# daysun/grid_ndt

Measured on NVIDIA B200. Metric: ndt_map_build_points_per_sec, higher is better.
Workload: dtype f64

## Files before the change

grid_ndt_b200/_lib.py:

```python
import ctypes as C
import os
import subprocess
import sys

from ._abi import Counts, NdtParams, Params, PointCloud2, Registration, XchgInfo, XchgView

HERE = os.path.dirname(os.path.abspath(__file__))
REPO = os.path.dirname(HERE)
LIB_PATH = os.environ.get("GNDT_LIB") or os.path.join(HERE, "libgndt.so")
SOURCES = [os.path.join(HERE, "csrc", f) for f in (
    "gndt_api.cu", "gndt_device.cuh", "gndt_sort.cuh", "gndt_reduce.cuh", "gndt_label.cuh", "gndt_update.cuh",
    "gndt_exchange.cuh", "gndt_graph.cuh", "gndt_scan.cuh", "gndt_ndt.cuh")]
HEADER = os.path.join(REPO, "include", "gndt.h")
LOOKUP_HEADER = os.path.join(REPO, "include", "gndt_lookup.h")

NVCC_FLAGS = ["-O3", "-std=c++17", "-gencode", "arch=compute_100a,code=sm_100a", "-lineinfo",
              "-Xcompiler", "-fPIC", "-shared"]


def build_library(force=False, verbose=False):
    deps = SOURCES + [HEADER, LOOKUP_HEADER]
    if not force and os.path.exists(LIB_PATH) and all(
            os.path.getmtime(LIB_PATH) >= os.path.getmtime(d) for d in deps if os.path.exists(d)):
        return LIB_PATH
    nvcc = os.environ.get("NVCC", "nvcc")
    cmd = [nvcc] + NVCC_FLAGS + ["-o", LIB_PATH, SOURCES[0], "-I" + os.path.join(REPO, "include")]
    if verbose:
        print(" ".join(cmd), file=sys.stderr)
    subprocess.check_call(cmd)
    return LIB_PATH


class GndtError(RuntimeError):
    def __init__(self, status, msg):
        super().__init__(f"gndt status {status}: {msg}")
        self.status = status


_lib = None

_vp, _sz, _i = C.c_void_p, C.c_size_t, C.c_int
SYMBOLS = {
    "gndt_version": (C.c_char_p, []),
    "gndt_last_error": (C.c_char_p, [_vp]),
    "gndt_default_params": (None, [C.POINTER(Params)]),
    "gndt_create": (_i, [C.POINTER(Params), _i, C.POINTER(_vp)]),
    "gndt_destroy": (_i, [_vp]),
    "gndt_set_params": (_i, [_vp, C.POINTER(Params)]),
    "gndt_build": (_i, [_vp, _vp, _sz, _sz, _i, _vp]),
    "gndt_build_msg": (_i, [_vp, C.POINTER(PointCloud2), _vp]),
    "gndt_update": (_i, [_vp, _vp, _sz, _sz, _i, _vp]),
    "gndt_remove": (_i, [_vp, _vp, _sz, _sz, _i, _vp]),
    "gndt_changed_columns": (_i, [_vp, _vp, _sz, _i, C.POINTER(_sz)]),
    "gndt_counts": (_i, [_vp, C.POINTER(Counts)]),
    "gndt_copy_voxels": (_i, [_vp, _vp, _sz, _i, C.POINTER(_sz)]),
    "gndt_copy_slopes": (_i, [_vp, _vp, _sz, _i, C.POINTER(_sz)]),
    "gndt_copy_columns": (_i, [_vp, _vp, _sz, _i, C.POINTER(_sz)]),
    "gndt_device_voxels": (_i, [_vp, C.POINTER(_vp), C.POINTER(_sz)]),
    "gndt_halo_pack": (_i, [_vp, _vp, _vp, _sz, _vp]),
    "gndt_halo_edges": (_i, [_vp, _vp, _vp, _vp]),
    "gndt_apply_strip_offsets": (_i, [_vp, _vp, C.POINTER(C.c_uint64), C.POINTER(C.c_uint32), C.POINTER(C.c_uint32), _i, _vp]),
    "gndt_device_count_ptr": (_i, [_vp, C.POINTER(_vp)]),
    "gndt_device_table_ptr": (_i, [_vp, C.POINTER(_vp), C.POINTER(_sz)]),
    "gndt_build_edges": (_i, [_vp, _vp, _sz, _vp, _sz, _vp]),
    "gndt_copy_edges": (_i, [_vp, _vp, _sz, _vp, _sz, _i, C.POINTER(_sz), C.POINTER(_sz)]),
    "gndt_xchg_create": (_i, [_vp, _i, _i, _sz, _sz, _i, C.POINTER(XchgInfo)]),
    "gndt_xchg_connect": (_i, [_vp, C.POINTER(XchgInfo), _i]),
    "gndt_xchg_run": (_i, [_vp, _vp]),
    "gndt_xchg_stage": (_i, [_vp, _vp]),
    "gndt_xchg_counts_ready": (_i, [_vp]),
    "gndt_xchg_send": (_i, [_vp, _vp]),
    "gndt_xchg_view_get": (_i, [_vp, C.POINTER(XchgView)]),
    "gndt_multi_create": (_i, [C.POINTER(Params), C.POINTER(C.c_int), _i, _sz, _sz, _i, C.POINTER(_vp)]),
    "gndt_multi_destroy": (_i, [_vp]),
    "gndt_multi_build": (_i, [_vp, _vp, _sz, _sz, _i]),
    "gndt_multi_update": (_i, [_vp, _vp, _sz, _sz, _i]),
    "gndt_multi_view": (_i, [_vp, _i, C.POINTER(XchgView)]),
    "gndt_multi_cuts": (_i, [_vp, C.POINTER(C.c_int32), _i]),
    "gndt_multi_handle": (_vp, [_vp, _i]),
    "gndt_multi_last_error": (C.c_char_p, [_vp]),
    "gndt_plan_tiles": (_i, [_vp, _vp, _sz, _sz, _i, _i, C.POINTER(C.c_int32), _vp]),
    "gndt_set_stage_timing": (_i, [_vp, _i]),
    "gndt_stage_ms": (_i, [_vp, C.POINTER(C.c_float)]),
    "gndt_launch_count": (_i, [_vp, C.POINTER(C.c_uint64)]),
    "gndt_fast_div_status": (_i, [_vp, C.POINTER(C.c_int), C.POINTER(C.c_uint64)]),
    "gndt_trans_morton_xyz": (_i, [C.POINTER(C.c_float), C.c_float, C.c_float, C.POINTER(C.c_float),
                                   C.POINTER(C.c_int32), C.POINTER(C.c_int32), C.POINTER(C.c_int32)]),
    "gndt_count_morton": (C.c_uint32, [C.c_uint32, C.c_uint32]),
    "gndt_morton_to_xy": (None, [C.c_uint32, C.POINTER(C.c_uint32), C.POINTER(C.c_uint32)]),
    "gndt_morton_string": (_i, [C.c_int32, C.c_int32, C.c_char_p]),
    "gndt_cell_center": (_i, [C.POINTER(C.c_float), C.c_float, C.c_float, C.c_int32, C.c_int32, C.c_int32,
                              C.POINTER(C.c_float)]),
    "gndt_origin": (_i, [_vp, C.POINTER(C.c_float)]),
    "gndt_default_ndt_params": (None, [C.POINTER(NdtParams)]),
    "gndt_register": (_i, [_vp, _vp, _sz, _sz, _i, C.POINTER(C.c_double), C.POINTER(NdtParams), C.POINTER(Registration), _vp]),
    "gndt_key_layout": (_i, [_vp, C.POINTER(C.c_int)]),
    "gndt_find_column": (C.c_int64, [_vp, _sz, C.c_int32, C.c_int32]),
    "gndt_find_slope": (C.c_int64, [_vp, _sz, _vp, C.c_int32, C.c_int32, C.c_int32]),
    "gndt_neighbor_column": (C.c_int64, [_vp, _sz, C.c_int32, C.c_int32, _i]),
}


def lib():
    global _lib
    if _lib is None:
        if not os.path.exists(LIB_PATH):
            raise GndtError(-2, f"{LIB_PATH} is not built (run __graft_entry__.build()); there is no CPU fallback")
        L = C.CDLL(LIB_PATH)
        for name, (res, args) in SYMBOLS.items():
            fn = getattr(L, name)
            fn.restype, fn.argtypes = res, args
        _lib = L
    return _lib
```

grid_ndt_b200/csrc/gndt_api.cu:

```cuda
#include <algorithm>
#include <cmath>
#include <cstdio>
#include <cstdlib>
#include <cstring>
#include <string>
#include <thread>
#include <vector>

#include "gndt_device.cuh"
#include "gndt_lookup.h"
#include "gndt_label.cuh"
#include "gndt_reduce.cuh"
#include "gndt_sort.cuh"
#include "gndt_update.cuh"
#include "gndt_exchange.cuh"
#include "gndt_graph.cuh"
#include "gndt_ndt.cuh"
#include <unistd.h>

using namespace gndt;

namespace {

thread_local std::string g_create_error;

struct Buffer {
  void *p = nullptr;
  size_t bytes = 0;
};

enum EvId { EV_H2D0, EV_START, EV_KEY, EV_SORT, EV_REDUCE, EV_LABEL, EV_EDGES, EV_COUNT };

struct DivCheck {
  float len = -1.f;
  float rinv = 0.f;
  int ok = 0;
};

struct SmallWords {
  Totals tot;
  u32 n_new;
  struct {
    int have[2];
    u32 done_counter;
  } x;
};
static_assert(sizeof(Totals) == 32 && sizeof(SmallWords) == 48, "SmallWords layout");

}

struct gndt_handle {
  int device = 0;
  gndt_params params;
  std::string err;
  Buffer in_stage, buf_a, buf_b, zero;
  Buffer mom, mom_alt, table, slopes, columns, vfirst, slope_col;
  void *ring = nullptr;
  cudaEvent_t ring_ev[4] = {};
  bool ring_used[4] = {};
  Buffer msg_points;
  Buffer mom_scan, upd_work;
  int pending_fuse = 0;
  size_t pending_points = 0;
  Ctl saved_ctl;
  gndt_params res_params;
  const u32 *changed_dev = nullptr, *changed_count_dev = nullptr;
  size_t n_changed = 0;
  bool n_changed_valid = false;
  Buffer small;
  size_t cap_points = 0, cap_voxels = 0;
  Ctl *ctl = nullptr;
  u32 *hist = nullptr;
  u32 *zhist = nullptr;
  u32 *row_start = nullptr, *row_end = nullptr;
  u32 *lb[2] = {nullptr, nullptr};
  u64 *glb[2] = {nullptr, nullptr};
  Buffer lookback;
  u64 *tile_state = nullptr;
  GroupState *tile_groups = nullptr;
  TileCarry *carry = nullptr;
  u64 *blk_state = nullptr;
  GroupState *blk_groups = nullptr;
  size_t zero_bytes_used = 0;
  size_t sort_tiles = 0, sort_groups = 0, red_tiles = 0, label_blocks = 0;
  Buffer f_zero;
  Buffer g_work, g_off, g_tgt;
  size_t g_slopes = 0, g_targets = 0;
  bool g_valid = false;
  Buffer ndt_vox, ndt_pts, ndt_part;
  double *ndt_host = nullptr;
  bool ndt_ready = false;
  Buffer xbuf;
  XLayout xl = {};
  XPeers xp = {};
  void *x_opened[kMaxRanks] = {};
  int x_what = 0;
  cudaStream_t x_stream = nullptr;
  cudaEvent_t x_ev[2] = {};
  cudaStream_t x_copy[2] = {};
  cudaEvent_t x_ev_counts = nullptr, x_ev_copy = nullptr;
  u32 *x_counts_host = nullptr;
  bool x_staged = false;
  u32 x_epoch = 0;
  bool x_created = false, x_connected = false;
  bool built = false;
  bool counts_valid = false;
  Ctl host_ctl;
  Totals host_tot, saved_tot;
  cudaStream_t last_stream = nullptr;
  cudaEvent_t ev[EV_COUNT] = {};
  bool timed_h2d = false;
  bool stage_timing = false;
  bool stages_valid = false;
  uint64_t launches = 0;
  uint64_t total_points = 0;
  int sm_count = 148;
  int sort_ctas_per_sm[2] = {1, 1};
  DivCheck div[2];
  uint64_t divcheck_values = 0;
};

namespace {

#define GNDT_CUDA(h, call)                                                                   \
  do {                                                                                       \
    cudaError_t e_ = (call);                                                                 \
    if (e_ != cudaSuccess) {                                                                 \
      (h)->err = std::string(#call) + ": " + cudaGetErrorString(e_);                         \
      return GNDT_ERR_CUDA;                                                                  \
    }                                                                                        \
  } while (0)

int ensure(gndt_handle *h, Buffer &b, size_t bytes) {
  if (b.bytes >= bytes) return GNDT_OK;
  if (b.p) GNDT_CUDA(h, cudaFree(b.p));
  b.p = nullptr;
  b.bytes = 0;
  GNDT_CUDA(h, cudaMalloc(&b.p, bytes));
  b.bytes = bytes;
  return GNDT_OK;
}

int ensure_keep(gndt_handle *h, Buffer &b, size_t bytes, size_t keep, cudaStream_t st) {
  if (b.bytes >= bytes) return GNDT_OK;
  void *np = nullptr;
  GNDT_CUDA(h, cudaMalloc(&np, bytes));
  if (b.p && keep) GNDT_CUDA(h, cudaMemcpyAsync(np, b.p, keep, cudaMemcpyDeviceToDevice, st));
  if (b.p) { GNDT_CUDA(h, cudaStreamSynchronize(st)); GNDT_CUDA(h, cudaFree(b.p)); }
  b.p = np;
  b.bytes = bytes;
  return GNDT_OK;
}

size_t align_up(size_t v, size_t a) { return (v + a - 1) / a * a; }

struct Layout {
  size_t bytes = 0;
  size_t take(size_t n) { const size_t o = bytes; bytes = align_up(bytes + n, 256); return o; }
};
template <typename T> T *at(const Buffer &b, size_t off) { return reinterpret_cast<T *>(static_cast<char *>(b.p) + off); }

struct ScanScratch {
  size_t ctl, state, groups;
  ScanScratch(Layout &L, size_t n) {
    const LookbackScratch s = lookback_scratch((n + kScanTile - 1) / kScanTile);
    ctl = L.take(sizeof(ScanCtl));
    state = L.take(s.words * sizeof(u64));
    groups = L.take(s.groups * sizeof(GroupState));
  }
};

template <typename... KArgs, typename... Args>
void launch(gndt_handle *h, bool pdl, void (*kernel)(KArgs...), dim3 grid, dim3 block, size_t smem, cudaStream_t st,
            Args &&...args) {
  cudaLaunchConfig_t cfg = {};
  cfg.gridDim = grid; cfg.blockDim = block; cfg.dynamicSmemBytes = smem; cfg.stream = st;
  cudaLaunchAttribute attr[1];
  attr[0].id = cudaLaunchAttributeProgrammaticStreamSerialization;
  attr[0].val.programmaticStreamSerializationAllowed = 1;
  cfg.attrs = attr;
  cfg.numAttrs = pdl ? 1 : 0;
  cudaLaunchKernelEx(&cfg, kernel, static_cast<KArgs>(args)...);
  h->launches += 1;
}

struct KeepLaunchCount {
  gndt_handle *h;
  uint64_t n;
  explicit KeepLaunchCount(gndt_handle *h_) : h(h_), n(h_->launches) {}
  ~KeepLaunchCount() { h->launches = n; }
};

int upload(gndt_handle *h, Buffer &stage, const void *xyz, size_t bytes, int mem, cudaStream_t st, cudaEvent_t h2d0,
           const float **d_in) {
  *d_in = static_cast<const float *>(xyz);
  if (mem != GNDT_MEM_HOST) return GNDT_OK;
  const int rc = ensure(h, stage, bytes);
  if (rc != GNDT_OK) return rc;
  if (h2d0) GNDT_CUDA(h, cudaEventRecord(h2d0, st));
  GNDT_CUDA(h, cudaMemcpyAsync(stage.p, xyz, bytes, cudaMemcpyHostToDevice, st));
  *d_in = static_cast<const float *>(stage.p);
  return GNDT_OK;
}

float max_abs_offset(float len) {
  auto ok = [len](uint32_t b) {
    float a;
    memcpy(&a, &b, 4);
    volatile float q = a / len;
    return std::ceil((float)q) <= (float)GNDT_MAX_INDEX;
  };
  uint32_t lo = 0, hi = 0x7f7fffffu;
  if (ok(hi)) lo = hi;
  while (lo + 1 < hi) {
    const uint32_t mid = lo + (hi - lo) / 2;
    if (ok(mid)) lo = mid; else hi = mid;
  }
  float a;
  memcpy(&a, &lo, 4);
  return a;
}

DevParams to_dev(const gndt_params &p, size_t cap_voxels) {
  DevParams d;
  d.max_abs[0] = max_abs_offset(p.grid_len);
  d.max_abs[1] = max_abs_offset(p.z_len);
  d.idx_offset = 0;
  d.fast_div = 0;
  d.rinv[0] = d.rinv[1] = 0.f;
  d.grid_len = p.grid_len; d.z_len = p.z_len; d.slope_interval = p.slope_interval;
  d.demand = p.demand; d.min_points = p.min_points;
  d.rough_max = p.rough_max; d.angle_max_deg = p.angle_max_deg; d.reach_height = p.reach_height;
  d.origin_first = p.origin_is_first_point;
  d.origin[0] = p.origin[0]; d.origin[1] = p.origin[1]; d.origin[2] = p.origin[2];
  d.normalize_cov = p.normalize_cov;
  d.tile_lo = p.tile_lo; d.tile_hi = p.tile_hi;
  d.max_voxels = (u32)cap_voxels;
  return d;
}

__global__ void divcheck_kernel(float len, u32 lo_bits, u32 hi_bits, float *rinv_out, unsigned long long *mismatches) {
  const float r = refined_rcp(len);
  if (blockIdx.x == 0 && threadIdx.x == 0) *rinv_out = r;
  unsigned long long bad = 0;
  for (u64 b = (u64)lo_bits + (u64)blockIdx.x * blockDim.x + threadIdx.x; b <= hi_bits; b += (u64)gridDim.x * blockDim.x) {
    const float a = __uint_as_float((u32)b);
    const float exact = ceilf(__fdiv_rn(a, len));
    const float fast = hoisted_div_ceil(a, len, r);
    if (!(exact == fast)) bad++;
  }
  if (bad) atomicAdd(mismatches, bad);
}

int verify_fast_div(gndt_handle *h, float len, DivCheck &out) {
  if (out.len == len) return GNDT_OK;
  out.len = len;
  out.ok = 0;
  out.rinv = 0.f;
  const char *force = getenv("GNDT_EXACT_DIV");
  if (force && force[0] == '1') return GNDT_OK;
  void *scratch = nullptr;
  GNDT_CUDA(h, cudaMalloc(&scratch, 64));
  GNDT_CUDA(h, cudaMemset(scratch, 0, 64));
  uint32_t lo, hi;
  const float top = 2.f * max_abs_offset(len);
  memcpy(&lo, &len, 4);
  memcpy(&hi, &top, 4);
  KeepLaunchCount keep(h);
  launch(h, false, divcheck_kernel, h->sm_count * 8, 256, 0, nullptr, len, lo, hi, (float *)scratch,
         (unsigned long long *)((char *)scratch + 8));
  unsigned long long host[2] = {0, 0};
  cudaError_t e = cudaGetLastError();
  if (e == cudaSuccess) e = cudaMemcpy(host, scratch, 16, cudaMemcpyDeviceToHost);
  cudaFree(scratch);
  if (e != cudaSuccess) { h->err = std::string("divcheck: ") + cudaGetErrorString(e); return GNDT_ERR_CUDA; }
  memcpy(&out.rinv, &host[0], 4);
  out.ok = (host[1] == 0) ? 1 : 0;
  h->divcheck_values += (uint64_t)hi - lo + 1;
  return GNDT_OK;
}

DevParams make_dev(gndt_handle *h, const gndt_params &p, size_t cap_voxels) {
  DevParams d = to_dev(p, cap_voxels);
  d.fast_div = (h->div[0].ok && h->div[1].ok && h->div[0].len == p.grid_len && h->div[1].len == p.z_len) ? 1 : 0;
  d.rinv[0] = h->div[0].rinv;
  d.rinv[1] = h->div[1].rinv;
  return d;
}

int validate_params(const gndt_params *p) {
  if (!p) return GNDT_ERR_INVALID_ARG;
  if (!(p->grid_len > 0.f) || !(p->z_len > 0.f) || !std::isfinite(p->grid_len) || !std::isfinite(p->z_len))
    return GNDT_ERR_INVALID_ARG;
  if (p->demand != GNDT_DEMAND_SLOPE && p->demand != GNDT_DEMAND_TRUE) return GNDT_ERR_INVALID_ARG;
  if (p->min_points < 1) return GNDT_ERR_INVALID_ARG;
  return GNDT_OK;
}

int reserve(gndt_handle *h, size_t n, size_t cap_vox, size_t keep_mom, cudaStream_t st) {
  int rc;
  if ((rc = ensure(h, h->buf_a, n * sizeof(float4))) != GNDT_OK) return rc;
  if ((rc = ensure(h, h->buf_b, n * sizeof(float4))) != GNDT_OK) return rc;
  if ((rc = ensure_keep(h, h->mom, cap_vox * sizeof(VoxMoments), keep_mom, st)) != GNDT_OK) return rc;
  if ((rc = ensure(h, h->table, cap_vox * sizeof(gndt_voxel))) != GNDT_OK) return rc;
  if ((rc = ensure(h, h->slopes, cap_vox * sizeof(gndt_slope))) != GNDT_OK) return rc;
  if ((rc = ensure(h, h->columns, cap_vox * sizeof(gndt_column))) != GNDT_OK) return rc;
  if ((rc = ensure(h, h->vfirst, cap_vox * sizeof(u32))) != GNDT_OK) return rc;
  if ((rc = ensure(h, h->slope_col, cap_vox * sizeof(u32))) != GNDT_OK) return rc;
  if ((rc = ensure(h, h->small, sizeof(SmallWords))) != GNDT_OK) return rc;
  h->cap_points = n;
  h->cap_voxels = cap_vox;
  h->sort_tiles = (n + kSortTile - 1) / kSortTile;
  h->sort_groups = (h->sort_tiles + kSortGroup - 1) / kSortGroup;
  h->red_tiles = (n + kRedTile - 1) / kRedTile;
  h->label_blocks = (cap_vox + kLabelThreads - 1) / kLabelThreads;
  const LookbackScratch red = lookback_scratch(h->red_tiles), fin = lookback_scratch(h->label_blocks);
  Layout Z;
  const size_t o_ctl = Z.take(sizeof(Ctl));
  const size_t o_hist = Z.take((size_t)kMaxPasses * kMaxBins * sizeof(u32));
  const size_t o_zh = Z.take(kZHistBins * sizeof(u32));
  const size_t o_rs = Z.take(65536 * sizeof(u32));
  const size_t o_re = Z.take(65536 * sizeof(u32));
  const size_t o_ts = Z.take(red.words * sizeof(u64));
  const size_t o_tg = Z.take(red.groups * sizeof(GroupState));
  const size_t o_ca = Z.take(h->red_tiles * sizeof(TileCarry));
  const size_t o_bs = Z.take(fin.words * sizeof(u64));
  const size_t o_bg = Z.take(fin.groups * sizeof(GroupState));
  if ((rc = ensure(h, h->zero, Z.bytes)) != GNDT_OK) return rc;
  h->ctl = at<Ctl>(h->zero, o_ctl);
  h->hist = at<u32>(h->zero, o_hist);
  h->zhist = at<u32>(h->zero, o_zh);
  h->row_start = at<u32>(h->zero, o_rs);
  h->row_end = at<u32>(h->zero, o_re);
  h->tile_state = at<u64>(h->zero, o_ts);
  h->tile_groups = at<GroupState>(h->zero, o_tg);
  h->carry = at<TileCarry>(h->zero, o_ca);
  h->blk_state = at<u64>(h->zero, o_bs);
  h->blk_groups = at<GroupState>(h->zero, o_bg);
  h->zero_bytes_used = Z.bytes;
  Layout B;
  const size_t lb_bytes = h->sort_tiles * kMaxBins * sizeof(u32) + 256, glb_bytes = h->sort_groups * kMaxBins * sizeof(u64) + 256;
  const size_t o_lb[2] = {B.take(lb_bytes), B.take(lb_bytes)}, o_glb[2] = {B.take(glb_bytes), B.take(glb_bytes)};
  if ((rc = ensure(h, h->lookback, B.bytes)) != GNDT_OK) return rc;
  for (int k = 0; k < 2; ++k) {
    h->lb[k] = at<u32>(h->lookback, o_lb[k]);
    h->glb[k] = at<u64>(h->lookback, o_glb[k]);
  }
  return GNDT_OK;
}

int grid_for(const gndt_handle *h, size_t work_items, int per_block, int max_waves) {
  size_t blocks = (work_items + per_block - 1) / per_block;
  size_t cap = (size_t)h->sm_count * max_waves;
  if (blocks > cap) blocks = cap;
  if (blocks < 1) blocks = 1;
  return (int)blocks;
}

int sync_counts(gndt_handle *h) {
  if (!h->built) { h->err = "no map has been built on this handle"; return GNDT_ERR_STATE; }
  if (h->counts_valid) return GNDT_OK;
  GNDT_CUDA(h, cudaMemcpyAsync(&h->host_ctl, h->ctl, sizeof(Ctl), cudaMemcpyDeviceToHost, h->last_stream));
  GNDT_CUDA(h, cudaMemcpyAsync(&h->host_tot, h->small.p, sizeof(Totals), cudaMemcpyDeviceToHost, h->last_stream));
  GNDT_CUDA(h, cudaStreamSynchronize(h->last_stream));
  if (h->pending_fuse) {
    const int sign = h->pending_fuse;
    h->pending_fuse = 0;
    if (h->host_ctl.err) {
      const u32 e = h->host_ctl.err;
      h->host_ctl = h->saved_ctl;
      h->host_tot = h->saved_tot;
      GNDT_CUDA(h, cudaMemcpyAsync(h->ctl, &h->saved_ctl, sizeof(Ctl), cudaMemcpyHostToDevice, h->last_stream));
      GNDT_CUDA(h, cudaMemcpyAsync(h->small.p, &h->saved_tot, sizeof(Totals), cudaMemcpyHostToDevice, h->last_stream));
      GNDT_CUDA(h, cudaStreamSynchronize(h->last_stream));
      h->counts_valid = true;
      if (e & kErrWatchdog) { h->err = "device watchdog tripped (look-back / TMA wait never resolved)"; return GNDT_ERR_INTERNAL; }
      if (e & kErrUnmatched) { h->err = "gndt_remove: the scan holds points that were never fused into the map; map unchanged"; return GNDT_ERR_STATE; }
      h->err = "voxel table capacity (max_voxels) exceeded; map unchanged";
      return GNDT_ERR_CAPACITY;
    }
    std::swap(h->mom, h->mom_alt);
    if (sign > 0) h->total_points += h->pending_points;
    else h->total_points -= h->pending_points;
    u32 nc = 0;
    GNDT_CUDA(h, cudaMemcpy(&nc, h->changed_count_dev, 4, cudaMemcpyDeviceToHost));
    h->n_changed = nc;
    h->n_changed_valid = true;
  }
  if (h->host_ctl.err & kErrWatchdog) { h->err = "device watchdog tripped (look-back / TMA wait never resolved)"; return GNDT_ERR_INTERNAL; }
  if (h->host_ctl.err & kErrCapacity) { h->err = "voxel table capacity (max_voxels) exceeded"; return GNDT_ERR_CAPACITY; }
  h->counts_valid = true;
  return GNDT_OK;
}

int front_end(gndt_handle *h, cudaStream_t st, const float *d_in, size_t n, size_t stride_f, size_t start,
              const DevParams &dp, VoxMoments *out) {
  GNDT_CUDA(h, cudaMemsetAsync(h->zero.p, 0, h->zero_bytes_used, st));
  const size_t tiles = (n + kSortTile - 1) / kSortTile, groups = (tiles + kSortGroup - 1) / kSortGroup;
  auto *bounds = dp.fast_div ? bounds_kernel<true> : bounds_kernel<false>;
  launch(h, true, bounds, grid_for(h, n, 256 * 4, 8), 256, 0, st, h->ctl, h->zhist, d_in, stride_f, n, start, (void *)h->lb[0],
         tiles * kFirstMaxBins * sizeof(u32), (void *)h->glb[0], groups * kFirstMaxBins * sizeof(u64), dp);
  launch(h, true, plan_kernel, 1, kZHistBins, 0, st, h->ctl, (const u32 *)h->zhist, h->hist);
  if (h->stage_timing) GNDT_CUDA(h, cudaEventRecord(h->ev[EV_KEY], st));
  float4 *A = static_cast<float4 *>(h->buf_a.p), *B = static_cast<float4 *>(h->buf_b.p);
  auto *first_pass = dp.fast_div ? sort_pass_kernel<true, true> : sort_pass_kernel<true, false>;
  auto *next_pass = dp.fast_div ? sort_pass_kernel<false, true> : sort_pass_kernel<false, false>;
  const int g0 = (int)std::min<size_t>(tiles, (size_t)h->sm_count * h->sort_ctas_per_sm[0]);
  const int g1 = (int)std::min<size_t>(tiles, (size_t)h->sm_count * h->sort_ctas_per_sm[1]);
  launch(h, true, first_pass, g0, kSortThreads, sizeof(SortSmem), st, h->ctl, 0, d_in, stride_f, n, start, (const float4 *)nullptr, A,
         h->lb[0], h->glb[0], h->lb[1], h->glb[1], h->hist, dp);
  for (int p = 1; p < kMaxPasses; ++p) {
    const float4 *src = (p & 1) ? A : B;
    float4 *dst = (p & 1) ? B : A;
    launch(h, true, next_pass, g1, kSortThreads, sizeof(SortSmem), st, h->ctl, p, (const float *)nullptr, (size_t)4, n, (size_t)0, src, dst,
           h->lb[p & 1], h->glb[p & 1], h->lb[(p + 1) & 1], h->glb[(p + 1) & 1], h->hist, dp);
  }
  if (h->stage_timing) GNDT_CUDA(h, cudaEventRecord(h->ev[EV_SORT], st));
  const int rtiles = (int)((n + kRedTile - 1) / kRedTile);
  auto *reduce = dp.fast_div ? reduce_kernel<true> : reduce_kernel<false>;
  launch(h, true, reduce, rtiles, kRedThreads, sizeof(RedSmem), st, h->ctl, (const float4 *)A, (const float4 *)B, out, h->carry,
         h->tile_state, h->tile_groups, dp);
  launch(h, true, fixup_kernel, grid_for(h, (size_t)rtiles * 32, 128, 16), 128, 0, st, h->ctl, out, (const TileCarry *)h->carry);
  if (h->stage_timing) GNDT_CUDA(h, cudaEventRecord(h->ev[EV_REDUCE], st));
  return GNDT_OK;
}

__global__ void table_bounds_kernel(Ctl *ctl, const gndt_voxel *table) {
  pdl_wait();
  pdl_trigger();
  const u32 n = ctl->n_voxels;
  if (threadIdx.x == 0 && n && !ctl->err) {
    ctl->cx_min = contiguous_index(table[0].sx);
    ctl->cx_max = contiguous_index(table[n - 1].sx);
  }
}

int back_end(gndt_handle *h, cudaStream_t st, const DevParams &dp, const VoxMoments *mom, bool bounds_from_table) {
  const int g_lab = grid_for(h, h->cap_voxels, kLabelThreads, 8);
  launch(h, true, finalize_label_kernel, g_lab, kFinThreads, sizeof(FinSmem), st, h->ctl, mom, (gndt_voxel *)h->table.p,
         (gndt_slope *)h->slopes.p, (gndt_column *)h->columns.p, (u32 *)h->vfirst.p, (u32 *)h->slope_col.p, h->blk_state, h->blk_groups,
         &h->ctl->ticket[7], dp);
  if (bounds_from_table) launch(h, true, table_bounds_kernel, 1, 32, 0, st, h->ctl, (const gndt_voxel *)h->table.p);
  launch(h, true, column_finish_kernel, g_lab, 256, 0, st, h->ctl, (const u32 *)h->vfirst.p, (gndt_column *)h->columns.p,
         h->row_start, h->row_end);
  if (h->stage_timing) GNDT_CUDA(h, cudaEventRecord(h->ev[EV_LABEL], st));
  launch(h, true, edges_kernel, g_lab, 256, 0, st, h->ctl, (gndt_voxel *)h->table.p, (gndt_slope *)h->slopes.p,
         (const gndt_column *)h->columns.p, (const u32 *)h->slope_col.p, (const u32 *)h->row_start, (const u32 *)h->row_end, dp);
  GNDT_CUDA(h, cudaEventRecord(h->ev[EV_EDGES], st));
  return GNDT_OK;
}

int check_cloud_args(gndt_handle *h, const void *xyz, size_t n, size_t stride_bytes, int mem, const char *who) {
  if (!xyz || n == 0 || stride_bytes < 12 || (stride_bytes & 3) || (mem != GNDT_MEM_HOST && mem != GNDT_MEM_DEVICE)) {
    h->err = std::string(who) + ": bad argument (xyz NULL, n == 0, stride not a multiple of 4 >= 12, or bad mem)";
    return GNDT_ERR_INVALID_ARG;
  }
  if (n > GNDT_MAX_POINTS) { h->err = std::string(who) + ": n exceeds GNDT_MAX_POINTS"; return GNDT_ERR_CAPACITY; }
  return GNDT_OK;
}

}

extern "C" {

const char *gndt_version(void) { return "gndt 0.3 (abi 2, sm_100a)"; }

const char *gndt_last_error(const gndt_handle *h) { return h ? h->err.c_str() : g_create_error.c_str(); }

void gndt_default_params(gndt_params *p) {
  if (!p) return;
  memset(p, 0, sizeof(*p));
  p->grid_len = 0.5f; p->z_len = 0.1f; p->slope_interval = 0.08f;
  p->demand = GNDT_DEMAND_SLOPE; p->min_points = 3;
  p->rough_max = 100.f; p->angle_max_deg = 30.f; p->reach_height = 0.15f;
  p->origin_is_first_point = 1;
}

int gndt_create(const gndt_params *params, int device, gndt_handle **out) {
  if (!out) return GNDT_ERR_INVALID_ARG;
  *out = nullptr;
  if (validate_params(params) != GNDT_OK) { g_create_error = "invalid gndt_params"; return GNDT_ERR_INVALID_ARG; }
  int n_dev = 0;
  cudaError_t e = cudaGetDeviceCount(&n_dev);
  if (e != cudaSuccess || device < 0 || device >= n_dev) {
    g_create_error = std::string("no usable CUDA device (there is no CPU fallback): ") +
                     (e != cudaSuccess ? cudaGetErrorString(e) : "device index out of range");
    return GNDT_ERR_CUDA;
  }
  gndt_handle *h = new gndt_handle();
  h->device = device;
  h->params = *params;
  if ((e = cudaSetDevice(device)) != cudaSuccess) { g_create_error = cudaGetErrorString(e); delete h; return GNDT_ERR_CUDA; }
  cudaDeviceGetAttribute(&h->sm_count, cudaDevAttrMultiProcessorCount, device);
  for (int i = 0; i < EV_COUNT; ++i)
    if ((e = cudaEventCreate(&h->ev[i])) != cudaSuccess) { g_create_error = cudaGetErrorString(e); delete h; return GNDT_ERR_CUDA; }
  e = cudaFuncSetAttribute(sort_pass_kernel<true, true>, cudaFuncAttributeMaxDynamicSharedMemorySize, (int)sizeof(SortSmem));
  if (e == cudaSuccess) e = cudaFuncSetAttribute(sort_pass_kernel<true, false>, cudaFuncAttributeMaxDynamicSharedMemorySize, (int)sizeof(SortSmem));
  if (e == cudaSuccess) e = cudaFuncSetAttribute(sort_pass_kernel<false, true>, cudaFuncAttributeMaxDynamicSharedMemorySize, (int)sizeof(SortSmem));
  if (e == cudaSuccess) e = cudaFuncSetAttribute(sort_pass_kernel<false, false>, cudaFuncAttributeMaxDynamicSharedMemorySize, (int)sizeof(SortSmem));
  if (e == cudaSuccess) e = cudaFuncSetAttribute(reduce_kernel<true>, cudaFuncAttributeMaxDynamicSharedMemorySize, (int)sizeof(RedSmem));
  if (e == cudaSuccess) e = cudaFuncSetAttribute(reduce_kernel<false>, cudaFuncAttributeMaxDynamicSharedMemorySize, (int)sizeof(RedSmem));
  if (e == cudaSuccess) e = cudaFuncSetAttribute(finalize_label_kernel, cudaFuncAttributeMaxDynamicSharedMemorySize, (int)sizeof(FinSmem));
  if (e != cudaSuccess) { g_create_error = std::string("kernel image for sm_100a not loadable on this device: ") + cudaGetErrorString(e); delete h; return GNDT_ERR_CUDA; }
  for (int k = 0; k < 2; ++k) {
    int nb = 0;
    e = k == 0 ? cudaOccupancyMaxActiveBlocksPerMultiprocessor(&nb, sort_pass_kernel<true, true>, kSortThreads, sizeof(SortSmem))
               : cudaOccupancyMaxActiveBlocksPerMultiprocessor(&nb, sort_pass_kernel<false, true>, kSortThreads, sizeof(SortSmem));
    if (e != cudaSuccess || nb < 1) { g_create_error = "partition pass kernel does not fit on this device"; delete h; return GNDT_ERR_CUDA; }
    h->sort_ctas_per_sm[k] = nb;
  }
  int rc = verify_fast_div(h, h->params.grid_len, h->div[0]);
  if (rc == GNDT_OK) rc = verify_fast_div(h, h->params.z_len, h->div[1]);
  if (rc != GNDT_OK) { g_create_error = h->err; delete h; return rc; }
  *out = h;
  return GNDT_OK;
}

int gndt_destroy(gndt_handle *h) {
  if (!h) return GNDT_ERR_INVALID_ARG;
  cudaSetDevice(h->device);
  for (int r = 0; r < kMaxRanks; ++r)
    if (h->x_opened[r]) cudaIpcCloseMemHandle(h->x_opened[r]);
  if (h->x_stream) { cudaStreamDestroy(h->x_stream); for (int i = 0; i < 2; ++i) if (h->x_ev[i]) cudaEventDestroy(h->x_ev[i]); }
  for (int i = 0; i < 2; ++i) if (h->x_copy[i]) cudaStreamDestroy(h->x_copy[i]);
  if (h->x_ev_counts) cudaEventDestroy(h->x_ev_counts);
  if (h->x_ev_copy) cudaEventDestroy(h->x_ev_copy);
  if (h->x_counts_host) cudaFreeHost(h->x_counts_host);
  if (h->ndt_host) cudaFreeHost(h->ndt_host);
  if (h->ring) { cudaFreeHost(h->ring); for (int i = 0; i < 4; ++i) if (h->ring_ev[i]) cudaEventDestroy(h->ring_ev[i]); }
  Buffer *bufs[] = {&h->in_stage, &h->buf_a, &h->buf_b, &h->zero, &h->mom, &h->mom_alt, &h->table, &h->slopes,
                    &h->columns, &h->vfirst, &h->slope_col, &h->mom_scan, &h->upd_work, &h->msg_points, &h->small, &h->lookback, &h->f_zero, &h->xbuf, &h->g_work, &h->g_off, &h->g_tgt,
                    &h->ndt_vox, &h->ndt_pts, &h->ndt_part};
  for (Buffer *b : bufs) if (b->p) cudaFree(b->p);
  for (int i = 0; i < EV_COUNT; ++i) if (h->ev[i]) cudaEventDestroy(h->ev[i]);
  delete h;
  return GNDT_OK;
}

int gndt_set_params(gndt_handle *h, const gndt_params *params) {
  if (!h || validate_params(params) != GNDT_OK) return GNDT_ERR_INVALID_ARG;
  h->params = *params;
  GNDT_CUDA(h, cudaSetDevice(h->device));
  int rc = verify_fast_div(h, h->params.grid_len, h->div[0]);
  if (rc == GNDT_OK) rc = verify_fast_div(h, h->params.z_len, h->div[1]);
  return rc;
}

static int build_device(gndt_handle *h, const float *d_in, size_t n, size_t stride_bytes, cudaStream_t st) {
  const size_t start = h->params.origin_is_first_point ? 1 : 0;
  const DevParams dp = make_dev(h, h->params, h->cap_voxels);
  h->ndt_ready = false;
  GNDT_CUDA(h, cudaEventRecord(h->ev[EV_START], st));
  int rc = front_end(h, st, d_in, n, stride_bytes / 4, start, dp, (VoxMoments *)h->mom.p);
  if (rc != GNDT_OK) return rc;
  launch(h, true, totals_kernel, 1, 32, 0, st, &static_cast<SmallWords *>(h->small.p)->tot, (const Ctl *)h->ctl, (u64)n, 1, 1);
  rc = back_end(h, st, dp, (const VoxMoments *)h->mom.p, false);
  if (rc != GNDT_OK) return rc;
  GNDT_CUDA(h, cudaGetLastError());
  h->built = true;
  h->pending_fuse = 0;
  h->n_changed_valid = false;
  h->res_params = h->params;
  h->stages_valid = h->stage_timing;
  h->total_points = n;
  h->last_stream = st;
  return GNDT_OK;
}

static int begin_build(gndt_handle *h, size_t n, cudaStream_t st) {
  GNDT_CUDA(h, cudaSetDevice(h->device));
  h->built = false;
  h->counts_valid = false;
  h->launches = 0;
  const size_t cap_vox = h->params.max_voxels ? (size_t)h->params.max_voxels : n;
  return reserve(h, n, cap_vox, 0, st);
}

int gndt_build(gndt_handle *h, const void *xyz, size_t n, size_t stride_bytes, int mem, void *stream) {
  if (!h) return GNDT_ERR_INVALID_ARG;
  int rc = check_cloud_args(h, xyz, n, stride_bytes, mem, "gndt_build");
  if (rc != GNDT_OK) return rc;
  cudaStream_t st = static_cast<cudaStream_t>(stream);
  if ((rc = begin_build(h, n, st)) != GNDT_OK) return rc;
  const float *d_in;
  h->timed_h2d = mem == GNDT_MEM_HOST;
  if ((rc = upload(h, h->in_stage, xyz, n * stride_bytes, mem, st, h->ev[EV_H2D0], &d_in)) != GNDT_OK) return rc;
  return build_device(h, d_in, n, stride_bytes, st);
}

__global__ void ingest_kernel(const unsigned char *raw, size_t n, u32 point_step, u32 xo, u32 yo, u32 zo, int big_endian, float4 *out) {
  for (size_t i = (size_t)blockIdx.x * blockDim.x + threadIdx.x; i < n; i += (size_t)gridDim.x * blockDim.x) {
    const unsigned char *p = raw + i * point_step;
    u32 w[3];
    const u32 offs[3] = {xo, yo, zo};
#pragma unroll
    for (int k = 0; k < 3; ++k) {
      const unsigned char *q = p + offs[k];
      w[k] = big_endian ? ((u32)q[0] << 24 | (u32)q[1] << 16 | (u32)q[2] << 8 | (u32)q[3])
                        : ((u32)q[3] << 24 | (u32)q[2] << 16 | (u32)q[1] << 8 | (u32)q[0]);
    }
    out[i] = make_float4(__uint_as_float(w[0]), __uint_as_float(w[1]), __uint_as_float(w[2]), 0.f);
  }
}

static int upload_pageable(gndt_handle *h, void *dst, const void *src, size_t bytes, cudaStream_t st) {
  constexpr size_t kChunk = 8u << 20;
  constexpr int kSlots = 4, kThreads = 4;
  if (!h->ring) {
    GNDT_CUDA(h, cudaHostAlloc(&h->ring, kChunk * kSlots, cudaHostAllocDefault));
    for (int i = 0; i < kSlots; ++i) GNDT_CUDA(h, cudaEventCreateWithFlags(&h->ring_ev[i], cudaEventDisableTiming));
  }
  size_t off = 0;
  for (int slot = 0; off < bytes; slot = (slot + 1) % kSlots) {
    const size_t len = std::min(kChunk, bytes - off);
    char *stage = static_cast<char *>(h->ring) + (size_t)slot * kChunk;
    if (h->ring_used[slot]) GNDT_CUDA(h, cudaEventSynchronize(h->ring_ev[slot]));
    const char *from = static_cast<const char *>(src) + off;
    std::thread workers[kThreads - 1];
    const size_t part = (len + kThreads - 1) / kThreads;
    for (int t = 1; t < kThreads; ++t)
      workers[t - 1] = std::thread([=] { if (t * part < len) memcpy(stage + t * part, from + t * part, std::min(part, len - t * part)); });
    memcpy(stage, from, std::min(part, len));
    for (auto &w : workers) w.join();
    GNDT_CUDA(h, cudaMemcpyAsync(static_cast<char *>(dst) + off, stage, len, cudaMemcpyHostToDevice, st));
    GNDT_CUDA(h, cudaEventRecord(h->ring_ev[slot], st));
    h->ring_used[slot] = true;
    off += len;
  }
  return GNDT_OK;
}

int gndt_build_msg(gndt_handle *h, const gndt_pointcloud2 *msg, void *stream) {
  if (!h || !msg) return GNDT_ERR_INVALID_ARG;
  const size_t n = (size_t)msg->width * msg->height;
  const u32 ps = msg->point_step;
  if (!msg->data || n == 0 || ps < 12 || msg->x_offset + 4 > ps || msg->y_offset + 4 > ps || msg->z_offset + 4 > ps) {
    h->err = "gndt_build_msg: empty message or x/y/z fields outside point_step";
    return GNDT_ERR_INVALID_ARG;
  }
  if (n > GNDT_MAX_POINTS) { h->err = "gndt_build_msg: width * height exceeds GNDT_MAX_POINTS"; return GNDT_ERR_CAPACITY; }
  cudaStream_t st = static_cast<cudaStream_t>(stream);
  int rc = begin_build(h, n, st);
  if (rc == GNDT_OK) rc = ensure(h, h->in_stage, n * ps);
  if (rc != GNDT_OK) return rc;
  GNDT_CUDA(h, cudaEventRecord(h->ev[EV_H2D0], st));
  if (msg->host_pinned) GNDT_CUDA(h, cudaMemcpyAsync(h->in_stage.p, msg->data, n * ps, cudaMemcpyHostToDevice, st));
  else if ((rc = upload_pageable(h, h->in_stage.p, msg->data, n * ps, st)) != GNDT_OK) return rc;
  h->timed_h2d = true;
  const bool direct = !msg->is_bigendian && (ps % 4 == 0) && (msg->x_offset % 4 == 0) && msg->y_offset == msg->x_offset + 4 &&
                      msg->z_offset == msg->x_offset + 8;
  if (direct) return build_device(h, reinterpret_cast<const float *>(static_cast<const char *>(h->in_stage.p) + msg->x_offset), n, ps, st);
  if ((rc = ensure(h, h->msg_points, n * sizeof(float4))) != GNDT_OK) return rc;
  launch(h, false, ingest_kernel, grid_for(h, n, 256, 8), 256, 0, st, static_cast<const unsigned char *>(h->in_stage.p), n, ps,
         msg->x_offset, msg->y_offset, msg->z_offset, msg->is_bigendian ? 1 : 0, static_cast<float4 *>(h->msg_points.p));
  return build_device(h, static_cast<const float *>(h->msg_points.p), n, sizeof(float4), st);
}

static int fuse_scan(gndt_handle *h, const void *xyz, size_t n, size_t stride_bytes, int mem, void *stream, int sign) {
  const char *who = sign > 0 ? "gndt_update" : "gndt_remove";
  if (!h) return GNDT_ERR_INVALID_ARG;
  int rc = check_cloud_args(h, xyz, n, stride_bytes, mem, who);
  if (rc != GNDT_OK) return rc;
  if ((rc = sync_counts(h)) != GNDT_OK) return rc;
  if (h->params.grid_len != h->res_params.grid_len || h->params.z_len != h->res_params.z_len ||
      h->params.tile_lo != h->res_params.tile_lo || h->params.tile_hi != h->res_params.tile_hi) {
    h->err = std::string(who) + ": grid_len / z_len / strip range differ from the resident map's (two key spaces cannot be fused)";
    return GNDT_ERR_STATE;
  }
  if (sign > 0 && h->total_points + n > 0xFFFFFFFFull) { h->err = "gndt_update: more than 2^32 points fused"; return GNDT_ERR_CAPACITY; }
  cudaStream_t st = static_cast<cudaStream_t>(stream);
  GNDT_CUDA(h, cudaSetDevice(h->device));
  const u32 n_res = h->host_ctl.n_voxels;
  const float origin[3] = {h->host_ctl.origin[0], h->host_ctl.origin[1], h->host_ctl.origin[2]};
  h->saved_ctl = h->host_ctl;
  h->saved_tot = h->host_tot;
  h->counts_valid = false;
  h->launches = 0;
  h->n_changed_valid = false;
  h->ndt_ready = false;

  size_t cap_vox = h->cap_voxels;
  const size_t need = (size_t)n_res + (sign > 0 ? n : 0);
  if (h->params.max_voxels == 0 && need > cap_vox) cap_vox = need + need / 2;
  rc = reserve(h, n > h->cap_points ? n : h->cap_points, cap_vox, (size_t)n_res * sizeof(VoxMoments), st);
  if (rc != GNDT_OK) return rc;
  if ((rc = ensure(h, h->mom_alt, cap_vox * sizeof(VoxMoments))) != GNDT_OK) return rc;
  if ((rc = ensure(h, h->mom_scan, n * sizeof(VoxMoments))) != GNDT_OK) return rc;
  Layout W;
  const size_t wn = (n + 1) * 4, wv = (cap_vox + 1) * 4;
  const size_t o_is_new = W.take(wn), o_new_pos = W.take(wn), o_order = W.take(wn), o_valid = W.take(wn), o_order_pos = W.take(wn),
               o_changed = W.take(wn), o_new_keys = W.take(n * 8);
  const size_t o_inv = W.take(wv), o_dead = W.take(wv), o_dead_pos = W.take(wv), o_touch_first = W.take(wv);
  const size_t scan_items = std::max(n, cap_vox);
  const ScanScratch sc[3] = {ScanScratch(W, scan_items), ScanScratch(W, scan_items), ScanScratch(W, scan_items)};
  if ((rc = ensure(h, h->upd_work, W.bytes)) != GNDT_OK) return rc;
  const Buffer &w = h->upd_work;
  u32 *is_new = at<u32>(w, o_is_new), *new_pos = at<u32>(w, o_new_pos), *order = at<u32>(w, o_order), *valid = at<u32>(w, o_valid),
      *order_pos = at<u32>(w, o_order_pos), *changed = at<u32>(w, o_changed);
  u64 *new_keys = at<u64>(w, o_new_keys);
  u32 *inv = at<u32>(w, o_inv), *dead = at<u32>(w, o_dead), *dead_pos = at<u32>(w, o_dead_pos), *touch_first = at<u32>(w, o_touch_first);
  auto exclusive_scan = [&](int k, const u32 *in, u32 n_fixed, const u32 *n_dev, u32 *out, size_t items) {
    launch(h, false, exclusive_scan_kernel, grid_for(h, (items + kScanTile - 1) / kScanTile, 1, 4), 256, 0, st, at<ScanCtl>(w, sc[k].ctl),
           in, n_fixed, n_dev, out, at<u64>(w, sc[k].state), at<GroupState>(w, sc[k].groups));
  };

  const float *d_in;
  h->timed_h2d = mem == GNDT_MEM_HOST;
  if ((rc = upload(h, h->in_stage, xyz, n * stride_bytes, mem, st, h->ev[EV_H2D0], &d_in)) != GNDT_OK) return rc;
  gndt_params p = h->params;
  p.origin_is_first_point = 0;
  p.origin[0] = origin[0]; p.origin[1] = origin[1]; p.origin[2] = origin[2];
  DevParams dp = make_dev(h, p, cap_vox);
  dp.idx_offset = sign > 0 ? (u32)h->total_points : 0u;

  GNDT_CUDA(h, cudaEventRecord(h->ev[EV_START], st));
  VoxMoments *res = (VoxMoments *)h->mom.p, *scan = (VoxMoments *)h->mom_scan.p, *merged = (VoxMoments *)h->mom_alt.p;
  rc = front_end(h, st, d_in, n, stride_bytes / 4, 0, dp, scan);
  if (rc != GNDT_OK) return rc;
  SmallWords *small = static_cast<SmallWords *>(h->small.p);
  launch(h, false, totals_kernel, 1, 32, 0, st, &small->tot, h->ctl, (u64)n, 0, sign);
  const int g_scan = grid_for(h, n, 256, 8), g_res = grid_for(h, std::max<size_t>(n_res, 1), 256, 8);
  GNDT_CUDA(h, cudaMemsetAsync(is_new, 0, o_order_pos - o_is_new, st));
  GNDT_CUDA(h, cudaMemsetAsync(dead, 0, o_touch_first - o_dead, st));
  GNDT_CUDA(h, cudaMemsetAsync(at<char>(w, sc[0].ctl), 0, W.bytes - sc[0].ctl, st));
  GNDT_CUDA(h, cudaMemsetAsync(inv, 0xFF, wv, st));
  GNDT_CUDA(h, cudaMemsetAsync(touch_first, 0xFF, wv, st));
  launch(h, false, update_match_kernel, g_scan, 256, 0, st, h->ctl, res, n_res, scan, sign, inv, is_new, dead);
  exclusive_scan(0, is_new, 0u, &h->ctl->n_voxels, new_pos, n);
  if (sign < 0) exclusive_scan(1, dead, n_res, nullptr, dead_pos, n_res);
  launch(h, false, update_new_keys_kernel, g_scan, 256, 0, st, h->ctl, scan, is_new, new_pos, new_keys);
  launch(h, false, update_prepare_kernel, 1, 32, 0, st, h->ctl, n_res, new_pos, sign < 0 ? dead_pos : nullptr, (u32)cap_vox, &small->n_new);
  launch(h, false, update_merge_resident_kernel, g_res, 256, 0, st, h->ctl, res, n_res, scan, sign, inv, new_keys, &small->n_new, dead,
         dead_pos, merged);
  if (sign > 0) launch(h, false, update_merge_new_kernel, g_scan, 256, 0, st, h->ctl, res, n_res, scan, is_new, new_pos, merged);
  rc = back_end(h, st, dp, merged, true);
  if (rc != GNDT_OK) return rc;
  launch(h, false, changed_mark_kernel, g_scan, 256, 0, st, h->ctl, scan, (const gndt_column *)h->columns.p, touch_first);
  launch(h, false, changed_order_kernel, grid_for(h, cap_vox, 256, 8), 256, 0, st, h->ctl, touch_first, dp.idx_offset, (u32)n, order, valid);
  exclusive_scan(2, valid, (u32)n, nullptr, order_pos, n);
  launch(h, false, changed_compact_kernel, g_scan, 256, 0, st, order, valid, order_pos, (u32)n, changed);
  GNDT_CUDA(h, cudaGetLastError());
  h->changed_dev = changed;
  h->changed_count_dev = &at<ScanCtl>(w, sc[2].ctl)->total;
  h->pending_fuse = sign;
  h->pending_points = n;
  h->stages_valid = h->stage_timing;
  h->last_stream = st;
  return GNDT_OK;
}

int gndt_update(gndt_handle *h, const void *xyz, size_t n, size_t stride_bytes, int mem, void *stream) {
  return fuse_scan(h, xyz, n, stride_bytes, mem, stream, +1);
}

int gndt_remove(gndt_handle *h, const void *xyz, size_t n, size_t stride_bytes, int mem, void *stream) {
  return fuse_scan(h, xyz, n, stride_bytes, mem, stream, -1);
}

int gndt_changed_columns(gndt_handle *h, uint32_t *idx, size_t cap, int dst_mem, size_t *n_out) {
  if (!h) return GNDT_ERR_INVALID_ARG;
  int rc = sync_counts(h);
  if (rc != GNDT_OK) return rc;
  if (!h->n_changed_valid) { h->err = "gndt_changed_columns: the last call on this handle was not a gndt_update / gndt_remove"; return GNDT_ERR_STATE; }
  if (n_out) *n_out = h->n_changed;
  if (!idx) return GNDT_OK;
  if (h->n_changed > cap) { h->err = "destination capacity too small"; return GNDT_ERR_CAPACITY; }
  if (h->n_changed)
    GNDT_CUDA(h, cudaMemcpy(idx, h->changed_dev, h->n_changed * 4, dst_mem == GNDT_MEM_HOST ? cudaMemcpyDeviceToHost : cudaMemcpyDeviceToDevice));
  return GNDT_OK;
}

int gndt_counts(gndt_handle *h, gndt_counts_t *out) {
  if (!h || !out) return GNDT_ERR_INVALID_ARG;
  int rc = sync_counts(h);
  if (rc != GNDT_OK) return rc;
  const Ctl &c = h->host_ctl;
  out->n_input = h->host_tot.n_points;
  out->n_binned = h->host_tot.n_valid;
  out->n_dropped = h->host_tot.n_dropped;
  out->n_outside_tile = h->host_tot.n_outside;
  out->n_columns = c.n_columns;
  out->n_voxels = c.n_voxels;
  out->n_fitted = c.n_fitted;
  out->n_slopes = c.n_slopes;
  return GNDT_OK;
}

static int copy_out(gndt_handle *h, void *dst, size_t cap, int dst_mem, size_t *n_out, const void *src, size_t n,
                    size_t rec) {
  if (!dst && n) return GNDT_ERR_INVALID_ARG;
  if (n > cap) { h->err = "destination capacity too small"; return GNDT_ERR_CAPACITY; }
  if (n) {
    GNDT_CUDA(h, cudaMemcpyAsync(dst, src, n * rec, dst_mem == GNDT_MEM_HOST ? cudaMemcpyDeviceToHost : cudaMemcpyDeviceToDevice,
                                 h->last_stream));
    GNDT_CUDA(h, cudaStreamSynchronize(h->last_stream));
  }
  if (n_out) *n_out = n;
  return GNDT_OK;
}

int gndt_copy_voxels(gndt_handle *h, gndt_voxel *dst, size_t cap, int dst_mem, size_t *n_out) {
  if (!h) return GNDT_ERR_INVALID_ARG;
  int rc = sync_counts(h);
  if (rc != GNDT_OK) return rc;
  return copy_out(h, dst, cap, dst_mem, n_out, h->table.p, h->host_ctl.n_voxels, sizeof(gndt_voxel));
}
int gndt_copy_slopes(gndt_handle *h, gndt_slope *dst, size_t cap, int dst_mem, size_t *n_out) {
  if (!h) return GNDT_ERR_INVALID_ARG;
  int rc = sync_counts(h);
  if (rc != GNDT_OK) return rc;
  return copy_out(h, dst, cap, dst_mem, n_out, h->slopes.p, h->host_ctl.n_slopes, sizeof(gndt_slope));
}
int gndt_copy_columns(gndt_handle *h, gndt_column *dst, size_t cap, int dst_mem, size_t *n_out) {
  if (!h) return GNDT_ERR_INVALID_ARG;
  int rc = sync_counts(h);
  if (rc != GNDT_OK) return rc;
  return copy_out(h, dst, cap, dst_mem, n_out, h->columns.p, h->host_ctl.n_columns, sizeof(gndt_column));
}

int gndt_device_voxels(gndt_handle *h, const gndt_voxel **dptr, size_t *n) {
  if (!h || !dptr || !n) return GNDT_ERR_INVALID_ARG;
  int rc = sync_counts(h);
  if (rc != GNDT_OK) return rc;
  *dptr = static_cast<const gndt_voxel *>(h->table.p);
  *n = h->host_ctl.n_voxels;
  return GNDT_OK;
}

int gndt_halo_pack(gndt_handle *h, gndt_voxel *first_row_out, gndt_voxel *last_row_out, size_t cap_records, void *stream) {
  if (!h || !first_row_out || !last_row_out || cap_records < 1) return GNDT_ERR_INVALID_ARG;
  if (!h->built) { h->err = "no map has been built on this handle"; return GNDT_ERR_STATE; }
  cudaStream_t st = static_cast<cudaStream_t>(stream);
  GNDT_CUDA(h, cudaSetDevice(h->device));
  launch(h, false, halo_pack_kernel, 2, 256, 0, st, h->ctl, (const gndt_voxel *)h->table.p, first_row_out, last_row_out,
         (u32)cap_records);
  GNDT_CUDA(h, cudaGetLastError());
  return GNDT_OK;
}

int gndt_halo_edges(gndt_handle *h, const gndt_voxel *from_prev, const gndt_voxel *from_next, void *stream) {
  if (!h) return GNDT_ERR_INVALID_ARG;
  if (!h->built) { h->err = "no map has been built on this handle"; return GNDT_ERR_STATE; }
  cudaStream_t st = static_cast<cudaStream_t>(stream);
  GNDT_CUDA(h, cudaSetDevice(h->device));
  const DevParams dp = make_dev(h, h->params, h->cap_voxels);
  launch(h, false, halo_edges_kernel, grid_for(h, h->cap_voxels, 256, 8), 256, 0, st, h->ctl, (gndt_voxel *)h->table.p,
         (gndt_slope *)h->slopes.p, from_prev, from_next, nullptr, dp);
  h->counts_valid = false;
  GNDT_CUDA(h, cudaGetLastError());
  return GNDT_OK;
}

int gndt_apply_strip_offsets(gndt_handle *h, gndt_voxel *table, const uint64_t *offsets, const uint32_t *col_offsets,
                             const uint32_t *slope_offsets, int n_strips, void *stream) {
  if (!h || !table || !offsets || !col_offsets || !slope_offsets || n_strips < 1) return GNDT_ERR_INVALID_ARG;
  cudaStream_t st = static_cast<cudaStream_t>(stream);
  GNDT_CUDA(h, cudaSetDevice(h->device));
  for (int r = 0; r < n_strips; ++r) {
    const uint64_t cnt = offsets[r + 1] - offsets[r];
    if (!cnt || (col_offsets[r] == 0 && slope_offsets[r] == 0)) continue;
    launch(h, false, strip_offsets_kernel, grid_for(h, cnt, 256, 8), 256, 0, st, table, offsets[r], cnt, col_offsets[r], slope_offsets[r]);
  }
  GNDT_CUDA(h, cudaGetLastError());
  return GNDT_OK;
}

int gndt_device_count_ptr(gndt_handle *h, const uint32_t **d_n_voxels) {
  if (!h || !d_n_voxels) return GNDT_ERR_INVALID_ARG;
  if (!h->built) { h->err = "no map has been built on this handle"; return GNDT_ERR_STATE; }
  *d_n_voxels = &h->ctl->n_voxels;
  return GNDT_OK;
}

int gndt_device_table_ptr(gndt_handle *h, const gndt_voxel **dptr, size_t *capacity) {
  if (!h || !dptr) return GNDT_ERR_INVALID_ARG;
  if (!h->built) { h->err = "no map has been built on this handle"; return GNDT_ERR_STATE; }
  *dptr = static_cast<const gndt_voxel *>(h->table.p);
  if (capacity) *capacity = h->cap_voxels;
  return GNDT_OK;
}

int gndt_build_edges(gndt_handle *h, const gndt_slope *slopes, size_t n_slopes, const gndt_column *columns, size_t n_columns,
                     void *stream) {
  if (!h || ((slopes == nullptr) != (columns == nullptr))) return GNDT_ERR_INVALID_ARG;
  cudaStream_t st = static_cast<cudaStream_t>(stream);
  GNDT_CUDA(h, cudaSetDevice(h->device));
  h->g_valid = false;
  int cx_lo = 0, cx_hi = 0, rc;
  if (!slopes) {
    if ((rc = sync_counts(h)) != GNDT_OK) return rc;
    slopes = static_cast<const gndt_slope *>(h->slopes.p);
    columns = static_cast<const gndt_column *>(h->columns.p);
    n_slopes = h->host_ctl.n_slopes;
    n_columns = h->host_ctl.n_columns;
    if (!st) st = h->last_stream;
  }
  if (n_slopes > 0xFFFFFFFEull || n_columns > 0xFFFFFFFEull) return GNDT_ERR_CAPACITY;
  if (n_columns) {
    gndt_column ends[2];
    GNDT_CUDA(h, cudaMemcpyAsync(&ends[0], columns, sizeof(gndt_column), cudaMemcpyDeviceToHost, st));
    GNDT_CUDA(h, cudaMemcpyAsync(&ends[1], columns + n_columns - 1, sizeof(gndt_column), cudaMemcpyDeviceToHost, st));
    GNDT_CUDA(h, cudaStreamSynchronize(st));
    cx_lo = ends[0].sx > 0 ? ends[0].sx - 1 : ends[0].sx;
    cx_hi = ends[1].sx > 0 ? ends[1].sx - 1 : ends[1].sx;
  }
  const int n_rows = cx_hi - cx_lo + 1;
  const u32 S = (u32)n_slopes, C = (u32)n_columns;
  Layout W;
  const ScanScratch sc(W, n_slopes);
  const size_t o_rs = W.take((size_t)n_rows * 4), o_re = W.take((size_t)n_rows * 4);
  const size_t zero_bytes = W.bytes;
  const size_t o_sc = W.take((n_slopes + 1) * 4), o_dg = W.take((n_slopes + 1) * 4);
  if ((rc = ensure(h, h->g_work, W.bytes)) != GNDT_OK) return rc;
  if ((rc = ensure(h, h->g_off, (n_slopes + 1) * 4)) != GNDT_OK) return rc;
  const Buffer &w = h->g_work;
  ScanCtl *g = at<ScanCtl>(w, sc.ctl);
  u32 *rs = at<u32>(w, o_rs), *re = at<u32>(w, o_re), *slope_col = at<u32>(w, o_sc), *deg = at<u32>(w, o_dg);
  GNDT_CUDA(h, cudaMemsetAsync(w.p, 0, zero_bytes, st));
  GNDT_CUDA(h, cudaMemsetAsync(h->g_off.p, 0, (n_slopes + 1) * 4, st));
  h->g_slopes = n_slopes;
  h->g_targets = 0;
  if (S && C) {
    const DevParams dp = make_dev(h, h->params, 0);
    const int grid_c = grid_for(h, C, 256, 8), grid_s = grid_for(h, S, 256, 8);
    launch(h, false, graph_prepare_kernel, grid_c, 256, 0, st, columns, C, cx_lo, slope_col, rs, re);
    launch(h, false, graph_edges_kernel<false>, grid_s, 256, 0, st, slopes, S, columns, C, slope_col, rs, re, cx_lo, n_rows, deg, nullptr,
           nullptr, dp);
    launch(h, false, exclusive_scan_kernel, grid_for(h, (n_slopes + kScanTile - 1) / kScanTile, 1, 4), 256, 0, st, g, deg, S, nullptr,
           (u32 *)h->g_off.p, at<u64>(w, sc.state), at<GroupState>(w, sc.groups));
    ScanCtl hg;
    GNDT_CUDA(h, cudaMemcpyAsync(&hg, g, sizeof(hg), cudaMemcpyDeviceToHost, st));
    GNDT_CUDA(h, cudaStreamSynchronize(st));
    if (hg.err) { h->err = "graph scan watchdog"; return GNDT_ERR_INTERNAL; }
    h->g_targets = hg.total;
    if ((rc = ensure(h, h->g_tgt, std::max<size_t>(hg.total, 1) * 4)) != GNDT_OK) return rc;
    launch(h, false, graph_edges_kernel<true>, grid_s, 256, 0, st, slopes, S, columns, C, slope_col, rs, re, cx_lo, n_rows, nullptr,
           (const u32 *)h->g_off.p, (u32 *)h->g_tgt.p, dp);
    GNDT_CUDA(h, cudaStreamSynchronize(st));
  }
  GNDT_CUDA(h, cudaGetLastError());
  h->g_valid = true;
  return GNDT_OK;
}

int gndt_copy_edges(gndt_handle *h, uint32_t *offsets, size_t cap_offsets, uint32_t *targets, size_t cap_targets, int dst_mem,
                    size_t *n_slopes, size_t *n_targets) {
  if (!h) return GNDT_ERR_INVALID_ARG;
  if (!h->g_valid) { h->err = "gndt_copy_edges: call gndt_build_edges first"; return GNDT_ERR_STATE; }
  if (n_slopes) *n_slopes = h->g_slopes;
  if (n_targets) *n_targets = h->g_targets;
  if (!offsets && !targets) return GNDT_OK;
  if (cap_offsets < h->g_slopes + 1 || cap_targets < h->g_targets || !offsets || (!targets && h->g_targets)) {
    h->err = "destination capacity too small";
    return GNDT_ERR_CAPACITY;
  }
  GNDT_CUDA(h, cudaSetDevice(h->device));
  const cudaMemcpyKind kind = dst_mem == GNDT_MEM_HOST ? cudaMemcpyDeviceToHost : cudaMemcpyDeviceToDevice;
  GNDT_CUDA(h, cudaMemcpy(offsets, h->g_off.p, (h->g_slopes + 1) * 4, kind));
  if (h->g_targets) GNDT_CUDA(h, cudaMemcpy(targets, h->g_tgt.p, h->g_targets * 4, kind));
  return GNDT_OK;
}

static_assert(sizeof(gndt_xchg_info) == 128, "gndt_xchg_info is 128 bytes");
static_assert(sizeof(cudaIpcMemHandle_t) == 64, "ipc handle size");
constexpr int kPushCtas = 48;

int gndt_xchg_create(gndt_handle *h, int rank, int world, size_t cap_records, size_t cap_halo_records, int what,
                     gndt_xchg_info *mine) {
  if (!h || !mine || world < 1 || world > kMaxRanks || rank < 0 || rank >= world || cap_records < 1 || cap_halo_records < 1 ||
      !(what & (GNDT_X_VOXELS | GNDT_X_SLOPES | GNDT_X_COLUMNS)))
    return GNDT_ERR_INVALID_ARG;
  if (cap_records > 0xFFFFFFFEull) return GNDT_ERR_CAPACITY;
  GNDT_CUDA(h, cudaSetDevice(h->device));
  XLayout L = {};
  Layout B;
  L.mail = B.take(sizeof(XMail));
  L.halo[0] = B.take((cap_halo_records + 1) * sizeof(gndt_voxel));
  L.halo[1] = B.take((cap_halo_records + 1) * sizeof(gndt_voxel));
  L.voxels = B.take((what & GNDT_X_VOXELS) ? cap_records * sizeof(gndt_voxel) : 0);
  L.slopes = B.take((what & GNDT_X_SLOPES) ? cap_records * sizeof(gndt_slope) : 0);
  L.columns = B.take((what & GNDT_X_COLUMNS) ? cap_records * sizeof(gndt_column) : 0);
  L.total = B.bytes;
  L.cap_records = cap_records;
  L.cap_halo = cap_halo_records;
  int rc;
  if ((rc = ensure(h, h->xbuf, L.total)) != GNDT_OK) return rc;
  if ((rc = ensure(h, h->small, sizeof(SmallWords))) != GNDT_OK) return rc;
  GNDT_CUDA(h, cudaMemset(h->xbuf.p, 0, sizeof(XMail)));
  GNDT_CUDA(h, cudaMemset(&static_cast<SmallWords *>(h->small.p)->x, 0, sizeof(SmallWords::x)));
  h->xl = L;
  h->xp = XPeers{};
  h->xp.rank = rank;
  h->xp.world = world;
  h->x_what = what;
  h->x_epoch = 0;
  h->x_created = true;
  h->x_connected = false;
  if (!h->x_stream) {
    int lo_p = 0, hi_p = 0;
    GNDT_CUDA(h, cudaDeviceGetStreamPriorityRange(&lo_p, &hi_p));
    GNDT_CUDA(h, cudaStreamCreateWithPriority(&h->x_stream, cudaStreamNonBlocking, hi_p));
    for (int i = 0; i < 2; ++i) GNDT_CUDA(h, cudaEventCreateWithFlags(&h->x_ev[i], cudaEventDisableTiming));
    for (int i = 0; i < 2; ++i) GNDT_CUDA(h, cudaStreamCreateWithFlags(&h->x_copy[i], cudaStreamNonBlocking));
    GNDT_CUDA(h, cudaEventCreateWithFlags(&h->x_ev_counts, cudaEventDisableTiming));
    GNDT_CUDA(h, cudaEventCreateWithFlags(&h->x_ev_copy, cudaEventDisableTiming));
    GNDT_CUDA(h, cudaHostAlloc(reinterpret_cast<void **>(&h->x_counts_host), kMaxRanks * 4 * sizeof(u32), cudaHostAllocDefault));
  }
  h->x_staged = false;
  memset(mine, 0, sizeof(*mine));
  cudaIpcMemHandle_t ipc;
  GNDT_CUDA(h, cudaIpcGetMemHandle(&ipc, h->xbuf.p));
  memcpy(mine->ipc_mem, &ipc, 64);
  mine->ptr = (uint64_t)(uintptr_t)h->xbuf.p;
  mine->bytes = L.total;
  mine->cap_records = cap_records;
  mine->cap_halo = cap_halo_records;
  mine->device = h->device;
  mine->pid = (int32_t)getpid();
  mine->what = what;
  mine->rank = rank;
  return GNDT_OK;
}

int gndt_xchg_connect(gndt_handle *h, const gndt_xchg_info *all, int world) {
  if (!h || !all) return GNDT_ERR_INVALID_ARG;
  if (!h->x_created || world != h->xp.world) { h->err = "gndt_xchg_connect: create the exchange first / world mismatch"; return GNDT_ERR_STATE; }
  GNDT_CUDA(h, cudaSetDevice(h->device));
  for (int r = 0; r < world; ++r) {
    const gndt_xchg_info &in = all[r];
    if (in.rank != r || in.bytes != h->xl.total || in.cap_records != h->xl.cap_records || in.cap_halo != h->xl.cap_halo || in.what != h->x_what) {
      h->err = "gndt_xchg_connect: rank " + std::to_string(r) + " has a different exchange layout";
      return GNDT_ERR_INVALID_ARG;
    }
    if (r == h->xp.rank) { h->xp.buf[r] = static_cast<unsigned char *>(h->xbuf.p); continue; }
    if (in.pid == (int32_t)getpid()) {
      if (in.device != h->device) {
        int can = 0;
        GNDT_CUDA(h, cudaDeviceCanAccessPeer(&can, h->device, in.device));
        if (!can) { h->err = "no peer access between devices " + std::to_string(h->device) + " and " + std::to_string(in.device); return GNDT_ERR_CUDA; }
        cudaError_t e = cudaDeviceEnablePeerAccess(in.device, 0);
        if (e != cudaSuccess && e != cudaErrorPeerAccessAlreadyEnabled) { h->err = cudaGetErrorString(e); return GNDT_ERR_CUDA; }
        cudaGetLastError();
      }
      h->xp.buf[r] = reinterpret_cast<unsigned char *>((uintptr_t)in.ptr);
    } else {
      cudaIpcMemHandle_t ipc;
      memcpy(&ipc, in.ipc_mem, 64);
      void *p = nullptr;
      GNDT_CUDA(h, cudaIpcOpenMemHandle(&p, ipc, cudaIpcMemLazyEnablePeerAccess));
      h->x_opened[r] = p;
      h->xp.buf[r] = static_cast<unsigned char *>(p);
    }
  }
  h->x_connected = true;
  return GNDT_OK;
}

static void xchg_front(gndt_handle *h, cudaStream_t st, u32 epoch) {
  const XPeers &X = h->xp;
  const XLayout &L = h->xl;
  int *have = static_cast<SmallWords *>(h->small.p)->x.have;
  const DevParams dp = make_dev(h, h->params, h->cap_voxels);
  unsigned char *mine = X.buf[X.rank];
  launch(h, false, xchg_publish_kernel, 1, 32, 0, st, h->ctl, X, L, epoch);
  launch(h, false, xchg_halo_send_kernel, 2, 256, 0, st, h->ctl, (const gndt_voxel *)h->table.p, X, L, epoch);
  launch(h, false, xchg_halo_wait_kernel, 1, 32, 0, st, h->ctl, X, L, epoch, have);
  launch(h, false, halo_edges_kernel, grid_for(h, h->cap_voxels, 256, 4), 256, 0, st, h->ctl, (gndt_voxel *)h->table.p,
         (gndt_slope *)h->slopes.p, reinterpret_cast<const gndt_voxel *>(mine + L.halo[0]),
         reinterpret_cast<const gndt_voxel *>(mine + L.halo[1]), have, dp);
}

static int xchg_check(gndt_handle *h, const char *who) {
  if (!h->built) { h->err = "no map has been built on this handle"; return GNDT_ERR_STATE; }
  if (!h->x_connected) { h->err = std::string(who) + ": exchange not connected"; return GNDT_ERR_STATE; }
  return GNDT_OK;
}

int gndt_xchg_run(gndt_handle *h, void *stream) {
  if (!h) return GNDT_ERR_INVALID_ARG;
  int rc = xchg_check(h, "gndt_xchg_run");
  if (rc != GNDT_OK) return rc;
  if (h->x_staged) { h->err = "gndt_xchg_run: a staged exchange is waiting for gndt_xchg_send"; return GNDT_ERR_STATE; }
  cudaStream_t st = static_cast<cudaStream_t>(stream);
  GNDT_CUDA(h, cudaSetDevice(h->device));
  const u32 epoch = ++h->x_epoch;
  const XPeers &X = h->xp;
  const XLayout &L = h->xl;
  u32 *done_counter = &static_cast<SmallWords *>(h->small.p)->x.done_counter;
  xchg_front(h, st, epoch);
  GNDT_CUDA(h, cudaEventRecord(h->x_ev[0], st));
  GNDT_CUDA(h, cudaStreamWaitEvent(h->x_stream, h->x_ev[0], 0));
  launch(h, false, xchg_push_kernel, kPushCtas, kPushThreads, 0, h->x_stream, h->ctl, (const gndt_voxel *)h->table.p,
         (const gndt_slope *)h->slopes.p, (const gndt_column *)h->columns.p, X, L, h->x_what, epoch, done_counter, 0);
  launch(h, false, xchg_wait_kernel, 1, 32, 0, h->x_stream, h->ctl, X, L, epoch);
  GNDT_CUDA(h, cudaEventRecord(h->x_ev[1], h->x_stream));
  GNDT_CUDA(h, cudaStreamWaitEvent(st, h->x_ev[1], 0));
  h->counts_valid = false;
  h->last_stream = st;
  GNDT_CUDA(h, cudaGetLastError());
  return GNDT_OK;
}

int gndt_xchg_stage(gndt_handle *h, void *stream) {
  if (!h) return GNDT_ERR_INVALID_ARG;
  int rc = xchg_check(h, "gndt_xchg_stage");
  if (rc != GNDT_OK) return rc;
  if (h->x_staged) { h->err = "gndt_xchg_stage: the previous staged exchange has not been sent"; return GNDT_ERR_STATE; }
  cudaStream_t st = static_cast<cudaStream_t>(stream);
  GNDT_CUDA(h, cudaSetDevice(h->device));
  const u32 epoch = ++h->x_epoch;
  const XPeers &X = h->xp;
  const XLayout &L = h->xl;
  u32 *done_counter = &static_cast<SmallWords *>(h->small.p)->x.done_counter;
  xchg_front(h, st, epoch);
  launch(h, false, xchg_push_kernel, kPushCtas, kPushThreads, 0, st, h->ctl, (const gndt_voxel *)h->table.p, (const gndt_slope *)h->slopes.p,
         (const gndt_column *)h->columns.p, X, L, h->x_what, epoch, done_counter, 1);
  const XMail *mail = reinterpret_cast<const XMail *>(X.buf[X.rank] + L.mail);
  GNDT_CUDA(h, cudaMemcpyAsync(h->x_counts_host, mail->counts[epoch & 1], kMaxRanks * 4 * sizeof(u32), cudaMemcpyDeviceToHost, st));
  GNDT_CUDA(h, cudaEventRecord(h->x_ev_counts, st));
  h->x_staged = true;
  h->counts_valid = false;
  h->last_stream = st;
  GNDT_CUDA(h, cudaGetLastError());
  return GNDT_OK;
}

int gndt_xchg_counts_ready(gndt_handle *h) {
  if (!h) return GNDT_ERR_INVALID_ARG;
  if (!h->x_staged) return 0;
  const cudaError_t e = cudaEventQuery(h->x_ev_counts);
  if (e == cudaSuccess) return 1;
  if (e == cudaErrorNotReady) return 0;
  h->err = cudaGetErrorString(e);
  return GNDT_ERR_CUDA;
}

int gndt_xchg_send(gndt_handle *h, void *stream) {
  if (!h) return GNDT_ERR_INVALID_ARG;
  if (!h->x_staged) { h->err = "gndt_xchg_send: nothing staged"; return GNDT_ERR_STATE; }
  cudaStream_t st = static_cast<cudaStream_t>(stream);
  GNDT_CUDA(h, cudaSetDevice(h->device));
  GNDT_CUDA(h, cudaEventSynchronize(h->x_ev_counts));
  h->x_staged = false;
  const u32 epoch = h->x_epoch;
  const XPeers &X = h->xp;
  const XLayout &L = h->xl;
  const int W = X.world;
  uint64_t off[3] = {0, 0, 0}, total = 0;
  for (int r = 0; r < W; ++r) {
    const u32 *c = h->x_counts_host + 4 * r;
    if (c[3] != epoch) { h->err = "gndt_xchg_send: strip " + std::to_string(r) + " never published its counts (watchdog)"; return GNDT_ERR_INTERNAL; }
    if (r < X.rank) for (int k = 0; k < 3; ++k) off[k] += c[k];
    total += c[0];
  }
  if (total > L.cap_records) { h->err = "gathered map exceeds the exchange capacity: " + std::to_string(total) + " > " + std::to_string(L.cap_records) + " records"; return GNDT_ERR_CAPACITY; }
  const u32 *own = h->x_counts_host + 4 * X.rank;
  struct { int bit; size_t base, rec; uint64_t first, n; } tab[3] = {
      {GNDT_X_VOXELS, L.voxels, sizeof(gndt_voxel), off[0], own[0]},
      {GNDT_X_SLOPES, L.slopes, sizeof(gndt_slope), off[2], own[2]},
      {GNDT_X_COLUMNS, L.columns, sizeof(gndt_column), off[1], own[1]}};
  for (int j = 0; j < 2; ++j) GNDT_CUDA(h, cudaStreamWaitEvent(h->x_copy[j], h->x_ev_counts, 0));
  int n_copies = 0;
  for (int d = 1; d < W; ++d) {
    const int p = (X.rank + d) % W;
    for (const auto &t : tab) {
      if (!(h->x_what & t.bit) || t.n == 0) continue;
      const size_t at = t.base + (size_t)t.first * t.rec;
      GNDT_CUDA(h, cudaMemcpyAsync(X.buf[p] + at, X.buf[X.rank] + at, (size_t)t.n * t.rec, cudaMemcpyDefault, h->x_copy[n_copies++ & 1]));
    }
  }
  for (int j = 0; j < 2; ++j) {
    GNDT_CUDA(h, cudaEventRecord(j ? h->x_ev_copy : h->x_ev[0], h->x_copy[j]));
    GNDT_CUDA(h, cudaStreamWaitEvent(h->x_stream, j ? h->x_ev_copy : h->x_ev[0], 0));
  }
  launch(h, false, xchg_done_kernel, 1, 32, 0, h->x_stream, X, L, epoch);
  launch(h, false, xchg_wait_kernel, 1, 32, 0, h->x_stream, h->ctl, X, L, epoch);
  GNDT_CUDA(h, cudaEventRecord(h->x_ev[1], h->x_stream));
  GNDT_CUDA(h, cudaStreamWaitEvent(st, h->x_ev[1], 0));
  h->counts_valid = false;
  h->last_stream = st;
  GNDT_CUDA(h, cudaGetLastError());
  return GNDT_OK;
}

int gndt_xchg_view_get(gndt_handle *h, gndt_xchg_view *out) {
  if (!h || !out) return GNDT_ERR_INVALID_ARG;
  if (!h->x_connected || h->x_epoch == 0) { h->err = "gndt_xchg_view_get: no exchange has run"; return GNDT_ERR_STATE; }
  int rc = sync_counts(h);
  if (rc != GNDT_OK) return rc;
  XMail mail;
  GNDT_CUDA(h, cudaMemcpy(&mail, h->xp.buf[h->xp.rank] + h->xl.mail, sizeof(XMail), cudaMemcpyDeviceToHost));
  memset(out, 0, sizeof(*out));
  unsigned char *mine = h->xp.buf[h->xp.rank];
  out->voxels = (h->x_what & GNDT_X_VOXELS) ? reinterpret_cast<const gndt_voxel *>(mine + h->xl.voxels) : nullptr;
  out->slopes = (h->x_what & GNDT_X_SLOPES) ? reinterpret_cast<const gndt_slope *>(mine + h->xl.slopes) : nullptr;
  out->columns = (h->x_what & GNDT_X_COLUMNS) ? reinterpret_cast<const gndt_column *>(mine + h->xl.columns) : nullptr;
  out->world = h->xp.world;
  const int par = h->x_epoch & 1;
  for (int r = 0; r < h->xp.world; ++r) {
    const u32 *c = mail.counts[par][r];
    if (c[3] != h->x_epoch || mail.done[par][r] != h->x_epoch) { h->err = "exchange incomplete (epoch mismatch)"; return GNDT_ERR_INTERNAL; }
    out->strip_voxels[r] = c[0];
    out->strip_columns[r] = c[1];
    out->strip_slopes[r] = c[2];
    out->n_voxels += c[0];
    out->n_columns += c[1];
    out->n_slopes += c[2];
  }
  return GNDT_OK;
}

struct gndt_multi {
  std::vector<gndt_handle *> h;
  std::vector<int> dev;
  std::vector<cudaStream_t> st;
  std::vector<Buffer> cloud;
  std::vector<int32_t> cuts;
  gndt_params params;
  bool planned = false;
  std::string err;
};

static int multi_fail(gndt_multi *m, int i, int rc, const char *what) {
  m->err = std::string(what) + " (device index " + std::to_string(i) + "): " + (i >= 0 && i < (int)m->h.size() && m->h[i] ? m->h[i]->err : g_create_error);
  return rc;
}

int gndt_multi_create(const gndt_params *params, const int *devices, int ndev, size_t cap_records, size_t cap_halo_records, int what,
                      gndt_multi **out) {
  if (!out || !params || !devices || ndev < 1 || ndev > kMaxRanks) return GNDT_ERR_INVALID_ARG;
  *out = nullptr;
  gndt_multi *m = new gndt_multi();
  m->params = *params;
  m->h.assign(ndev, nullptr);
  m->dev.assign(devices, devices + ndev);
  m->st.assign(ndev, nullptr);
  m->cloud.resize(ndev);
  std::vector<gndt_xchg_info> info(ndev);
  for (int i = 0; i < ndev; ++i) {
    int rc = gndt_create(params, devices[i], &m->h[i]);
    if (rc == GNDT_OK && cudaStreamCreateWithFlags(&m->st[i], cudaStreamNonBlocking) != cudaSuccess) rc = GNDT_ERR_CUDA;
    if (rc == GNDT_OK) rc = gndt_xchg_create(m->h[i], i, ndev, cap_records, cap_halo_records, what, &info[i]);
    if (rc != GNDT_OK) { g_create_error = "gndt_multi_create: device " + std::to_string(devices[i]) + ": " + (m->h[i] ? m->h[i]->err : g_create_error); gndt_multi_destroy(m); return rc; }
  }
  for (int i = 0; i < ndev; ++i) {
    const int rc = gndt_xchg_connect(m->h[i], info.data(), ndev);
    if (rc != GNDT_OK) { g_create_error = "gndt_multi_create: " + m->h[i]->err; gndt_multi_destroy(m); return rc; }
  }
  *out = m;
  return GNDT_OK;
}

int gndt_multi_destroy(gndt_multi *m) {
  if (!m) return GNDT_ERR_INVALID_ARG;
  for (size_t i = 0; i < m->h.size(); ++i) {
    if (!m->h[i]) continue;
    cudaSetDevice(m->dev[i]);
    cudaDeviceSynchronize();
    if (m->cloud[i].p) cudaFree(m->cloud[i].p);
    if (m->st[i]) cudaStreamDestroy(m->st[i]);
    gndt_destroy(m->h[i]);
  }
  delete m;
  return GNDT_OK;
}

const char *gndt_multi_last_error(const gndt_multi *m) { return m ? m->err.c_str() : g_create_error.c_str(); }
gndt_handle *gndt_multi_handle(gndt_multi *m, int index) { return (m && index >= 0 && index < (int)m->h.size()) ? m->h[index] : nullptr; }

static int multi_stage(gndt_multi *m, const void *xyz, size_t n, size_t stride_bytes, int mem) {
  const size_t bytes = n * stride_bytes;
  for (size_t i = 0; i < m->h.size(); ++i) {
    gndt_handle *h = m->h[i];
    if (cudaSetDevice(m->dev[i]) != cudaSuccess) return multi_fail(m, (int)i, GNDT_ERR_CUDA, "cudaSetDevice");
    if (mem == GNDT_MEM_DEVICE && i == 0) continue;
    int rc = ensure(h, m->cloud[i], bytes);
    if (rc != GNDT_OK) return multi_fail(m, (int)i, rc, "cloud staging");
    cudaError_t e = mem == GNDT_MEM_HOST ? cudaMemcpyAsync(m->cloud[i].p, xyz, bytes, cudaMemcpyHostToDevice, m->st[i])
                                         : cudaMemcpyPeerAsync(m->cloud[i].p, m->dev[i], xyz, m->dev[0], bytes, m->st[i]);
    if (e != cudaSuccess) { h->err = cudaGetErrorString(e); return multi_fail(m, (int)i, GNDT_ERR_CUDA, "cloud copy"); }
  }
  return GNDT_OK;
}
static const void *multi_cloud(gndt_multi *m, size_t i, const void *xyz, int mem) { return (mem == GNDT_MEM_DEVICE && i == 0) ? xyz : m->cloud[i].p; }

int gndt_multi_build(gndt_multi *m, const void *xyz, size_t n, size_t stride_bytes, int mem) {
  if (!m || !xyz || n == 0) return GNDT_ERR_INVALID_ARG;
  const int nd = (int)m->h.size();
  int rc = multi_stage(m, xyz, n, stride_bytes, mem);
  if (rc != GNDT_OK) return rc;
  cudaSetDevice(m->dev[0]);
  m->cuts.assign(nd + 1, 0);
  gndt_params p0 = m->params;
  p0.tile_lo = p0.tile_hi = 0;
  if ((rc = gndt_set_params(m->h[0], &p0)) != GNDT_OK) return multi_fail(m, 0, rc, "set_params");
  if ((rc = gndt_plan_tiles(m->h[0], multi_cloud(m, 0, xyz, mem), n, stride_bytes, GNDT_MEM_DEVICE, nd, m->cuts.data(), m->st[0])) != GNDT_OK)
    return multi_fail(m, 0, rc, "gndt_plan_tiles");
  m->planned = true;
  for (int i = 0; i < nd; ++i) {
    cudaSetDevice(m->dev[i]);
    gndt_params p = m->params;
    const bool empty = nd > 1 && m->cuts[i] >= m->cuts[i + 1];
    p.tile_lo = nd == 1 ? 0 : (empty ? GNDT_MAX_INDEX : m->cuts[i]);
    p.tile_hi = nd == 1 ? 0 : (empty ? GNDT_MAX_INDEX + 1 : m->cuts[i + 1]);
    if ((rc = gndt_set_params(m->h[i], &p)) != GNDT_OK) return multi_fail(m, i, rc, "set_params");
    if ((rc = gndt_build(m->h[i], multi_cloud(m, i, xyz, mem), n, stride_bytes, GNDT_MEM_DEVICE, m->st[i])) != GNDT_OK) return multi_fail(m, i, rc, "gndt_build");
    if ((rc = gndt_xchg_run(m->h[i], m->st[i])) != GNDT_OK) return multi_fail(m, i, rc, "gndt_xchg_run");
  }
  return GNDT_OK;
}

int gndt_multi_update(gndt_multi *m, const void *xyz, size_t n, size_t stride_bytes, int mem) {
  if (!m || !xyz || n == 0) return GNDT_ERR_INVALID_ARG;
  if (!m->planned) { m->err = "gndt_multi_update: no map has been built"; return GNDT_ERR_STATE; }
  int rc = multi_stage(m, xyz, n, stride_bytes, mem);
  if (rc != GNDT_OK) return rc;
  for (size_t i = 0; i < m->h.size(); ++i) {
    cudaSetDevice(m->dev[i]);
    if ((rc = gndt_update(m->h[i], multi_cloud(m, i, xyz, mem), n, stride_bytes, GNDT_MEM_DEVICE, m->st[i])) != GNDT_OK) return multi_fail(m, (int)i, rc, "gndt_update");
    if ((rc = gndt_xchg_run(m->h[i], m->st[i])) != GNDT_OK) return multi_fail(m, (int)i, rc, "gndt_xchg_run");
  }
  return GNDT_OK;
}

int gndt_multi_view(gndt_multi *m, int index, gndt_xchg_view *out) {
  if (!m || !out || index < 0 || index >= (int)m->h.size()) return GNDT_ERR_INVALID_ARG;
  for (size_t i = 0; i < m->h.size(); ++i) {
    cudaSetDevice(m->dev[i]);
    gndt_xchg_view v;
    const int rc = gndt_xchg_view_get(m->h[i], (int)i == index ? out : &v);
    if (rc != GNDT_OK) return multi_fail(m, (int)i, rc, "exchange");
  }
  return GNDT_OK;
}

int gndt_multi_cuts(gndt_multi *m, int32_t *cuts, int cap) {
  if (!m || !cuts || cap < (int)m->cuts.size()) return GNDT_ERR_INVALID_ARG;
  std::copy(m->cuts.begin(), m->cuts.end(), cuts);
  return GNDT_OK;
}

__global__ void cx_hist_kernel(u32 *hist, const float *in, size_t stride_f, size_t n_in, size_t start, DevParams P) {
  float o[3];
  if (P.origin_first) { o[0] = __ldg(in); o[1] = __ldg(in + 1); o[2] = __ldg(in + 2); }
  else { o[0] = P.origin[0]; o[1] = P.origin[1]; o[2] = P.origin[2]; }
  const bool vec = (stride_f == 4) && ((reinterpret_cast<uintptr_t>(in) & 15) == 0);
  for (size_t i = start + (size_t)blockIdx.x * blockDim.x + threadIdx.x; i < n_in; i += (size_t)gridDim.x * blockDim.x) {
    float4 p = load_point(in, stride_f, i, vec);
    int cx, cy, cz;
    if (point_indices(p.x, p.y, p.z, o, P, cx, cy, cz)) atomicAdd(&hist[cx + kIdxBias], 1u);
  }
}

int gndt_plan_tiles(gndt_handle *h, const void *xyz, size_t n, size_t stride_bytes, int mem, int ntiles, int32_t *cuts,
                    void *stream) {
  if (!h || !xyz || !cuts || ntiles < 1 || n == 0 || stride_bytes < 12 || (stride_bytes & 3)) return GNDT_ERR_INVALID_ARG;
  cudaStream_t st = static_cast<cudaStream_t>(stream);
  GNDT_CUDA(h, cudaSetDevice(h->device));
  const float *d_in;
  int rc = upload(h, h->in_stage, xyz, n * stride_bytes, mem, st, nullptr, &d_in);
  if (rc != GNDT_OK) return rc;
  if ((rc = ensure(h, h->f_zero, 65536 * sizeof(u32) + 1024)) != GNDT_OK) return rc;
  GNDT_CUDA(h, cudaMemsetAsync(h->f_zero.p, 0, 65536 * sizeof(u32), st));
  const DevParams dp = make_dev(h, h->params, 0);
  launch(h, false, cx_hist_kernel, grid_for(h, n, 256 * 8, 8), 256, 0, st, (u32 *)h->f_zero.p, d_in, stride_bytes / 4, n,
         h->params.origin_is_first_point ? 1 : 0, dp);
  GNDT_CUDA(h, cudaGetLastError());
  u32 *hist = (u32 *)malloc(65536 * sizeof(u32));
  cudaError_t e = cudaMemcpyAsync(hist, h->f_zero.p, 65536 * sizeof(u32), cudaMemcpyDeviceToHost, st);
  if (e == cudaSuccess) e = cudaStreamSynchronize(st);
  if (e != cudaSuccess) { free(hist); h->err = cudaGetErrorString(e); return GNDT_ERR_CUDA; }
  uint64_t total = 0;
  for (int i = 0; i < 65536; ++i) total += hist[i];
  cuts[0] = -kIdxBias;
  cuts[ntiles] = kIdxBias;
  uint64_t acc = 0;
  int t = 1;
  for (int i = 0; i < 65536 && t < ntiles; ++i) {
    acc += hist[i];
    while (t < ntiles && acc * (uint64_t)ntiles >= total * (uint64_t)t) cuts[t++] = i - kIdxBias + 1;
  }
  for (; t < ntiles; ++t) cuts[t] = kIdxBias;
  free(hist);
  return GNDT_OK;
}

int gndt_set_stage_timing(gndt_handle *h, int on) {
  if (!h) return GNDT_ERR_INVALID_ARG;
  h->stage_timing = on != 0;
  return GNDT_OK;
}

int gndt_stage_ms(gndt_handle *h, float ms[GNDT_N_STAGES]) {
  if (!h || !ms) return GNDT_ERR_INVALID_ARG;
  if (!h->built) return GNDT_ERR_STATE;
  GNDT_CUDA(h, cudaStreamSynchronize(h->last_stream));
  for (int i = 0; i < GNDT_N_STAGES; ++i) ms[i] = 0.f;
  if (h->stages_valid) {
    GNDT_CUDA(h, cudaEventElapsedTime(&ms[GNDT_STAGE_KEY], h->ev[EV_START], h->ev[EV_KEY]));
    GNDT_CUDA(h, cudaEventElapsedTime(&ms[GNDT_STAGE_SORT], h->ev[EV_KEY], h->ev[EV_SORT]));
    GNDT_CUDA(h, cudaEventElapsedTime(&ms[GNDT_STAGE_REDUCE], h->ev[EV_SORT], h->ev[EV_REDUCE]));
    GNDT_CUDA(h, cudaEventElapsedTime(&ms[GNDT_STAGE_LABEL], h->ev[EV_REDUCE], h->ev[EV_LABEL]));
    GNDT_CUDA(h, cudaEventElapsedTime(&ms[GNDT_STAGE_EDGES], h->ev[EV_LABEL], h->ev[EV_EDGES]));
  }
  GNDT_CUDA(h, cudaEventElapsedTime(&ms[GNDT_STAGE_TOTAL], h->ev[EV_START], h->ev[EV_EDGES]));
  if (h->timed_h2d) GNDT_CUDA(h, cudaEventElapsedTime(&ms[GNDT_STAGE_H2D], h->ev[EV_H2D0], h->ev[EV_START]));
  return GNDT_OK;
}

int gndt_fast_div_status(gndt_handle *h, int *enabled, uint64_t *values_checked) {
  if (!h) return GNDT_ERR_INVALID_ARG;
  if (enabled) *enabled = (h->div[0].ok && h->div[1].ok) ? 1 : 0;
  if (values_checked) *values_checked = h->divcheck_values;
  return GNDT_OK;
}

int gndt_launch_count(gndt_handle *h, uint64_t *n_launches) {
  if (!h || !n_launches) return GNDT_ERR_INVALID_ARG;
  *n_launches = h->launches;
  return GNDT_OK;
}


static int host_axis(float p, float p0, float len, int32_t *s) {
  volatile float d = p - p0;
  volatile float q = std::fabs(d) / len;
  float c = std::ceil(q);
  if (!(c <= (float)GNDT_MAX_INDEX)) return 0;
  int32_t n = (int32_t)c;
  if (n == 0) n = 1;
  *s = (p > p0) ? n : -n;
  return 1;
}

int gndt_trans_morton_xyz(const float origin[3], float grid_len, float z_len, const float pos[3], int32_t *sx,
                          int32_t *sy, int32_t *sz) {
  if (!origin || !pos || !sx || !sy || !sz) return GNDT_ERR_INVALID_ARG;
  if (!host_axis(pos[0], origin[0], grid_len, sx) || !host_axis(pos[1], origin[1], grid_len, sy) ||
      !host_axis(pos[2], origin[2], z_len, sz))
    return GNDT_ERR_INVALID_ARG;
  return GNDT_OK;
}

uint32_t gndt_count_morton(uint32_t nx, uint32_t ny) {
  uint32_t m = 0;
  for (int k = 0; k < 16; ++k) m |= ((nx >> k) & 1u) << (2 * k + 1) | ((ny >> k) & 1u) << (2 * k);
  return m;
}

void gndt_morton_to_xy(uint32_t morton, uint32_t *nx, uint32_t *ny) {
  uint32_t a = 0, b = 0;
  for (int k = 0; k < 16; ++k) { a |= ((morton >> (2 * k + 1)) & 1u) << k; b |= ((morton >> (2 * k)) & 1u) << k; }
  if (nx) *nx = a;
  if (ny) *ny = b;
}

int gndt_morton_string(int32_t sx, int32_t sy, char *buf) {
  if (!buf) return 0;
  const char q = sx > 0 ? (sy > 0 ? 'A' : 'B') : (sy > 0 ? 'C' : 'D');
  return snprintf(buf, 16, "%c%d", q, (int)gndt_count_morton((uint32_t)abs(sx), (uint32_t)abs(sy)));
}

int gndt_cell_center(const float origin[3], float grid_len, float z_len, int32_t sx, int32_t sy, int32_t sz,
                     float center[3]) {
  if (!origin || !center || sx == 0 || sy == 0 || sz == 0) return GNDT_ERR_INVALID_ARG;
  const double ax = (std::abs(sx) - 0.5) * grid_len, ay = (std::abs(sy) - 0.5) * grid_len, az = (std::abs(sz) - 0.5) * z_len;
  center[0] = (float)(sx > 0 ? ax + origin[0] : origin[0] - ax);
  center[1] = (float)(sy > 0 ? ay + origin[1] : origin[1] - ay);
  center[2] = (float)(sz > 0 ? origin[2] + az : origin[2] - az);
  return GNDT_OK;
}

int gndt_key_layout(gndt_handle *h, int out[4]) {
  if (!h || !out) return GNDT_ERR_INVALID_ARG;
  int rc = sync_counts(h);
  if (rc != GNDT_OK) return rc;
  out[0] = h->host_ctl.n_passes; out[1] = h->host_ctl.bcol; out[2] = (int)h->host_ctl.ny; out[3] = h->host_ctl.bz;
  return GNDT_OK;
}

int64_t gndt_find_column(const gndt_column *cols, size_t n_cols, int32_t sx, int32_t sy) {
  return gndtl_find_column(cols, n_cols, sx, sy);
}
int64_t gndt_find_slope(const gndt_column *cols, size_t n_cols, const gndt_slope *slopes, int32_t sx, int32_t sy,
                        int32_t sz) {
  return gndtl_find_slope(cols, n_cols, slopes, sx, sy, sz);
}
int64_t gndt_neighbor_column(const gndt_column *cols, size_t n_cols, int32_t sx, int32_t sy, int dir) {
  return gndtl_neighbor_column(cols, n_cols, sx, sy, dir);
}

int gndt_origin(gndt_handle *h, float origin[3]) {
  if (!h || !origin) return GNDT_ERR_INVALID_ARG;
  int rc = sync_counts(h);
  if (rc != GNDT_OK) return rc;
  for (int i = 0; i < 3; ++i) origin[i] = h->host_ctl.origin[i];
  return GNDT_OK;
}


void gndt_default_ndt_params(gndt_ndt_params *p) {
  if (!p) return;
  memset(p, 0, sizeof(*p));
  p->outlier_ratio = 0.55f;
  p->min_voxel_points = 6;
  p->max_iterations = 100;
  p->translation_epsilon = 1e-4;
  p->rotation_epsilon = 1e-4;
}

namespace {

struct NdtEval {
  double score, g[6], H[36], c[3];
  uint64_t n_points, n_matched, n_pairs;
};

void so3_exp(const double phi[3], double E[9]) {
  const double th2 = phi[0] * phi[0] + phi[1] * phi[1] + phi[2] * phi[2], th = std::sqrt(th2);
  const double a = th2 < 1e-24 ? 1.0 - th2 / 6.0 : std::sin(th) / th;
  const double b = th2 < 1e-24 ? 0.5 - th2 / 24.0 : (1.0 - std::cos(th)) / th2;
  const double K[9] = {0.0, -phi[2], phi[1], phi[2], 0.0, -phi[0], -phi[1], phi[0], 0.0};
  for (int i = 0; i < 3; ++i)
    for (int j = 0; j < 3; ++j) {
      double kk = 0.0;
      for (int m = 0; m < 3; ++m) kk += K[3 * i + m] * K[3 * m + j];
      E[3 * i + j] = (i == j ? 1.0 : 0.0) + a * K[3 * i + j] + b * kk;
    }
}

bool chol6(const double A_in[36], const double b[6], double x[6]) {
  double L[36] = {};
  for (int i = 0; i < 6; ++i)
    for (int j = 0; j <= i; ++j) {
      double s = A_in[6 * i + j];
      for (int k = 0; k < j; ++k) s -= L[6 * i + k] * L[6 * j + k];
      if (i == j) {
        if (!(s > 0.0) || !std::isfinite(s)) return false;
        L[6 * i + i] = std::sqrt(s);
      } else {
        L[6 * i + j] = s / L[6 * j + j];
      }
    }
  double y[6];
  for (int i = 0; i < 6; ++i) {
    double s = b[i];
    for (int k = 0; k < i; ++k) s -= L[6 * i + k] * y[k];
    y[i] = s / L[6 * i + i];
  }
  for (int i = 5; i >= 0; --i) {
    double s = y[i];
    for (int k = i + 1; k < 6; ++k) s -= L[6 * k + i] * x[k];
    x[i] = s / L[6 * i + i];
  }
  return true;
}

int ndt_check_args(gndt_handle *h, const double *T, const gndt_ndt_params *np) {
  for (int i = 0; i < 16; ++i)
    if (!std::isfinite(T[i])) { h->err = "gndt_register: the guess is not finite"; return GNDT_ERR_INVALID_ARG; }
  if (T[12] != 0.0 || T[13] != 0.0 || T[14] != 0.0 || T[15] != 1.0) { h->err = "gndt_register: the guess's bottom row is not 0 0 0 1"; return GNDT_ERR_INVALID_ARG; }
  for (int i = 0; i < 3; ++i)
    for (int j = 0; j < 3; ++j) {
      const double rtr = T[i] * T[j] + T[4 + i] * T[4 + j] + T[8 + i] * T[8 + j];
      if (!(std::fabs(rtr - (i == j ? 1.0 : 0.0)) <= 1e-6)) { h->err = "gndt_register: the guess's rotation is not orthonormal"; return GNDT_ERR_INVALID_ARG; }
    }
  if (!(np->outlier_ratio > 0.f && np->outlier_ratio < 1.f) || np->min_voxel_points < 3 || np->max_iterations < 0 || np->reserved != 0 ||
      !(np->translation_epsilon >= 0.0) || !(np->rotation_epsilon >= 0.0) || !std::isfinite(np->translation_epsilon) ||
      !std::isfinite(np->rotation_epsilon)) {
    h->err = "gndt_register: ndt parameter out of range";
    return GNDT_ERR_INVALID_ARG;
  }
  return GNDT_OK;
}

}

int gndt_register(gndt_handle *h, const void *xyz, size_t n, size_t stride_bytes, int mem, const double guess[16],
                  const gndt_ndt_params *np, gndt_registration *out, void *stream) {
  if (!h) return GNDT_ERR_INVALID_ARG;
  if (!guess || !np || !out) { h->err = "gndt_register: guess, np and out must not be NULL"; return GNDT_ERR_INVALID_ARG; }
  int rc = check_cloud_args(h, xyz, n, stride_bytes, mem, "gndt_register");
  if (rc != GNDT_OK) return rc;
  if ((rc = ndt_check_args(h, guess, np)) != GNDT_OK) return rc;
  GNDT_CUDA(h, cudaSetDevice(h->device));
  if ((rc = sync_counts(h)) != GNDT_OK) return rc;
  KeepLaunchCount keep(h);
  cudaStream_t st = static_cast<cudaStream_t>(stream);
  const gndt_params &rp = h->res_params;
  const u32 n_vox = h->host_ctl.n_voxels, n_cols = h->host_ctl.n_columns;

  if (!h->ndt_ready) {
    if ((rc = ensure(h, h->ndt_vox, std::max<size_t>(n_vox, 1) * sizeof(NdtVoxel))) != GNDT_OK) return rc;
    launch(h, false, ndt_prepare_kernel, grid_for(h, n_vox, 256, 8), 256, 0, st, h->ctl, (const gndt_voxel *)h->table.p,
           (NdtVoxel *)h->ndt_vox.p, rp.normalize_cov);
  }
  const float *d_in;
  if ((rc = upload(h, h->ndt_pts, xyz, n * stride_bytes, mem, st, nullptr, &d_in)) != GNDT_OK) return rc;
  const int blocks = grid_for(h, n, kNdtThreads, 8);
  if ((rc = ensure(h, h->ndt_part, ((size_t)blocks + 1) * kNdtWidth * sizeof(double))) != GNDT_OK) return rc;
  if (!h->ndt_host) GNDT_CUDA(h, cudaHostAlloc(&h->ndt_host, kNdtWidth * sizeof(double), cudaHostAllocDefault));
  double *part = static_cast<double *>(h->ndt_part.p), *dres = part + (size_t)blocks * kNdtWidth;
  const size_t stride_f = stride_bytes / 4;

  launch(h, false, ndt_mean_kernel, blocks, kNdtThreads, 0, st, d_in, stride_f, n, part);
  launch(h, false, ndt_finish_kernel, 1, 32, 0, st, part, blocks, 4, dres);
  GNDT_CUDA(h, cudaGetLastError());
  GNDT_CUDA(h, cudaMemcpyAsync(h->ndt_host, dres, 4 * sizeof(double), cudaMemcpyDeviceToHost, st));
  GNDT_CUDA(h, cudaStreamSynchronize(st));
  h->ndt_ready = true;
  const uint64_t n_points = (uint64_t)h->ndt_host[3];
  const double pbar[3] = {n_points ? h->ndt_host[0] / (double)n_points : 0.0, n_points ? h->ndt_host[1] / (double)n_points : 0.0,
                          n_points ? h->ndt_host[2] / (double)n_points : 0.0};

  NdtPose P = {};
  {
    const double p_o = np->outlier_ratio, V = (double)rp.grid_len * (double)rp.grid_len * (double)rp.z_len;
    const double c1 = 10.0 * (1.0 - p_o), c2 = p_o / V, d3 = -std::log(c2);
    P.d1 = -std::log(c1 + c2) - d3;
    P.d2 = -2.0 * std::log((-std::log(c1 * std::exp(-0.5) + c2) - d3) / P.d1);
  }
  for (int i = 0; i < 3; ++i) P.origin[i] = h->host_ctl.origin[i];
  P.grid_len = rp.grid_len;
  P.z_len = rp.z_len;
  P.min_points = (u32)np->min_voxel_points;

  auto eval = [&](const double T[16], NdtEval &e) -> int {
    for (int i = 0; i < 3; ++i) {
      for (int j = 0; j < 3; ++j) P.r[3 * i + j] = T[4 * i + j];
      P.t[i] = T[4 * i + 3];
      P.c[i] = T[4 * i] * pbar[0] + T[4 * i + 1] * pbar[1] + T[4 * i + 2] * pbar[2] + T[4 * i + 3];
    }
    launch(h, false, ndt_pass_kernel, blocks, kNdtThreads, 0, st, d_in, stride_f, n, (const NdtVoxel *)h->ndt_vox.p,
           (const gndt_column *)h->columns.p, n_cols, P, part);
    launch(h, false, ndt_finish_kernel, 1, 32, 0, st, part, blocks, kNdtWidth, dres);
    GNDT_CUDA(h, cudaGetLastError());
    GNDT_CUDA(h, cudaMemcpyAsync(h->ndt_host, dres, kNdtWidth * sizeof(double), cudaMemcpyDeviceToHost, st));
    GNDT_CUDA(h, cudaStreamSynchronize(st));
    const double *r = h->ndt_host;
    e.score = r[0];
    for (int k = 0; k < 6; ++k) e.g[k] = r[1 + k];
    for (int k = 0, idx = 7; k < 6; ++k)
      for (int l = k; l < 6; ++l, ++idx) e.H[6 * k + l] = e.H[6 * l + k] = r[idx];
    for (int i = 0; i < 3; ++i) e.c[i] = P.c[i];
    e.n_points = (uint64_t)r[28];
    e.n_matched = (uint64_t)r[29];
    e.n_pairs = (uint64_t)r[30];
    return GNDT_OK;
  };

  double T[16];
  memcpy(T, guess, sizeof(T));
  NdtEval cur;
  if ((rc = eval(T, cur)) != GNDT_OK) return rc;
  int term = GNDT_NDT_MAX_ITER;
  uint32_t iters = 0;
  if (cur.n_pairs == 0) {
    term = GNDT_NDT_NO_MATCH;
    cur.score = 0.0;
    memset(cur.g, 0, sizeof(cur.g));
    memset(cur.H, 0, sizeof(cur.H));
  } else {
    constexpr double kLambda0 = 1e-3, kLambdaMin = 1e-12, kLambdaMax = 1e12;
    double lambda = kLambda0;
    while (iters < (uint32_t)np->max_iterations) {
      double hmax = 0.0;
      for (int i = 0; i < 6; ++i) hmax = std::max(hmax, std::fabs(cur.H[7 * i]));
      const double tiny = std::max(1e-6 * hmax, 1e-300);
      double A[36], delta[6];
      for (int i = 0; i < 36; ++i) A[i] = -cur.H[i];
      for (int i = 0; i < 6; ++i) A[7 * i] += lambda * std::max(-cur.H[7 * i], tiny);
      if (!chol6(A, cur.g, delta)) {
        lambda *= 10.0;
        if (lambda > kLambdaMax) { term = GNDT_NDT_STALLED; break; }
        continue;
      }
      const double dr = std::sqrt(delta[0] * delta[0] + delta[1] * delta[1] + delta[2] * delta[2]);
      const double dp = std::sqrt(delta[3] * delta[3] + delta[4] * delta[4] + delta[5] * delta[5]);
      if (lambda < 1.0 && dr < np->translation_epsilon && dp < np->rotation_epsilon) { term = GNDT_NDT_CONVERGED; break; }
      double E[9], Tn[16];
      so3_exp(delta + 3, E);
      memcpy(Tn, T, sizeof(Tn));
      for (int i = 0; i < 3; ++i) {
        double tt = cur.c[i] + delta[i];
        for (int j = 0; j < 3; ++j) {
          Tn[4 * i + j] = E[3 * i] * T[j] + E[3 * i + 1] * T[4 + j] + E[3 * i + 2] * T[8 + j];
          tt += E[3 * i + j] * (T[4 * j + 3] - cur.c[j]);
        }
        Tn[4 * i + 3] = tt;
      }
      NdtEval cand;
      if ((rc = eval(Tn, cand)) != GNDT_OK) return rc;
      ++iters;
      if (cand.score > cur.score) {
        memcpy(T, Tn, sizeof(T));
        cur = cand;
        lambda = std::max(lambda / 10.0, kLambdaMin);
      } else {
        lambda *= 10.0;
        if (lambda > kLambdaMax) { term = GNDT_NDT_STALLED; break; }
      }
    }
  }
  memset(out, 0, sizeof(*out));
  memcpy(out->pose, T, sizeof(T));
  memcpy(out->center, cur.c, sizeof(cur.c));
  out->score = cur.score;
  memcpy(out->gradient, cur.g, sizeof(cur.g));
  memcpy(out->hessian, cur.H, sizeof(cur.H));
  out->n_points = n_points;
  out->n_matched = cur.n_matched;
  out->n_pairs = cur.n_pairs;
  out->iterations = iters;
  out->termination = term;
  return GNDT_OK;
}

}
```

grid_ndt_b200/csrc/gndt_label.cuh:

```cuda
#pragma once
#include "gndt_device.cuh"
#include "gndt_reduce.cuh"

namespace gndt {

constexpr int kLabelThreads = 256;

__device__ __forceinline__ int contiguous_index(int s) { return s > 0 ? s - 1 : s; }

struct __align__(128) FinSmem {
  VoxMoments in[kLabelThreads + 2];
  float4 out[kLabelThreads * 6];
  unsigned long long mbar;
  u64 prefix;
  u32 warp_sums[32];
  u32 tile, total;
};

constexpr int kFinThreads = kLabelThreads + 32;
constexpr int kFinMinBlocks = 3;
__global__ void __launch_bounds__(kFinThreads, kFinMinBlocks)
finalize_label_kernel(Ctl *ctl, const VoxMoments *mom, gndt_voxel *table, gndt_slope *slopes,
                      gndt_column *columns, u32 *vfirst, u32 *slope_col, u64 *blk_state, GroupState *blk_groups, u32 *counters,
                      DevParams P) {
  pdl_wait();
  pdl_trigger();
  extern __shared__ __align__(128) unsigned char smem_fin[];
  FinSmem &S = *reinterpret_cast<FinSmem *>(smem_fin);
  const int tid = threadIdx.x;
  const bool helper = tid >= kLabelThreads;
  if (ctl->err) return;
  const u32 V = ctl->n_voxels;
  const u32 n_blocks = (V + kLabelThreads - 1) / kLabelThreads;
  const float o[3] = {ctl->origin[0], ctl->origin[1], ctl->origin[2]};
  auto mean_z = [&](const VoxMoments &r) { return (float)(r.m[2] + anchor_axis((u32)r.key & 0xFFFFu, o[2], P.z_len)); };
  if (tid == 0) mbar_init(&S.mbar, 1);
  for (u32 it = 0;; ++it) {
    __syncthreads();
    if (tid == 0) S.tile = atomicAdd(&counters[0], 1u);
    __syncthreads();
    const u32 blk = S.tile;
    if (blk >= n_blocks) return;
    const u32 v0 = blk * kLabelThreads;
    const u32 cnt = min((u32)kLabelThreads, V - v0);
    if (tid == 0) {
      const u32 lo = v0 > 0 ? v0 - 1 : 0, hi = min(v0 + cnt + 1, V);
      tma_load_1d(&S.in[lo + 1 - v0], mom + lo, (hi - lo) * (u32)sizeof(VoxMoments), &S.mbar);
    }
    if (!mbar_wait(&S.mbar, it & 1)) atomicOr(&ctl->err, kErrWatchdog);
    const u32 v = v0 + tid;
    const bool live = !helper && tid < (int)cnt;

    u64 key = 0;
    u32 count = 0, first = 0, flags = 0;
    float mz = 0.f;
    bool head = false, fitted = false;
    if (live) {
      const VoxMoments &me = S.in[tid + 1];
      key = me.key; count = me.count; first = me.first;
      fitted = (int)count >= P.min_points;
      mz = mean_z(me);
      const bool has_lo = (v > 0) && (S.in[tid].key >> 16) == (key >> 16);
      const bool has_hi = (v + 1 < V) && (S.in[tid + 2].key >> 16) == (key >> 16);
      head = !has_lo;
      if (fitted) {
        flags = GNDT_F_FITTED;
        bool up = false, down = false;
        const bool ordered = (P.demand == GNDT_DEMAND_SLOPE);
        if (has_hi && (S.in[tid + 2].key & 0xFFFFu) == (key & 0xFFFFu) + 1) {
          const VoxMoments &hi = S.in[tid + 2];
          const bool seen = (int)hi.count >= P.min_points && (!ordered || hi.first < first);
          up = fabsf(__fsub_rn(seen ? mean_z(hi) : 0.f, mz)) > P.slope_interval;
        }
        if (ordered && has_lo && (S.in[tid].key & 0xFFFFu) + 1 == (key & 0xFFFFu)) {
          const VoxMoments &lo = S.in[tid];
          const bool seen = (int)lo.count >= P.min_points && lo.first < first;
          down = fabsf(__fsub_rn(seen ? mean_z(lo) : 0.f, mz)) > P.slope_interval;
        }
        if (up) flags |= GNDT_F_UP;
        if (down) flags |= GNDT_F_DOWN;
        if (P.demand == GNDT_DEMAND_TRUE || !up) flags |= GNDT_F_SLOPE;
      }
      if (head) flags |= GNDT_F_COLUMN_HEAD;
    }
    const bool slope = (flags & GNDT_F_SLOPE) != 0;
    const u32 packed = ((head ? 1u : 0u) << 16) | (slope ? 1u : 0u);
    const u32 exc = block_exclusive_scan(packed, S.warp_sums);
    if (tid == kLabelThreads - 1) S.total = exc + packed;
    __syncthreads();

    if (helper) {
      const u32 total = S.total;
      const u64 pre = warp_lookback_grouped(blk_state, blk_groups, (int)blk, total >> 16, total & 0xFFFFu, &ctl->err);
      if (tid == kLabelThreads) {
        S.prefix = pre;
        if (blk == n_blocks - 1) {
          const u64 incl = pre + pack_pair(total >> 16, total & 0xFFFFu);
          ctl->n_columns = (u32)(incl >> 31);
          ctl->n_slopes = (u32)(incl & 0x7FFFFFFFu);
        }
      }
    } else if (live) {
      float f[24];
#pragma unroll
      for (int i = 0; i < 24; ++i) f[i] = 0.f;
      u32 *u = reinterpret_cast<u32 *>(f);
      const int cx = (int)(u32)(key >> 32) - kIdxBias, cy = (int)((u32)(key >> 16) & 0xFFFFu) - kIdxBias,
                cz = (int)((u32)key & 0xFFFFu) - kIdxBias;
      u[0] = (u32)signed_index(cx); u[1] = (u32)signed_index(cy); u[2] = (u32)signed_index(cz);
      u[3] = count; u[4] = first;
      if (fitted) {
        const VoxMoments &me = S.in[tid + 1];
        f[5] = (float)(me.m[0] + anchor_axis((u32)(key >> 32), o[0], P.grid_len));
        f[6] = (float)(me.m[1] + anchor_axis((u32)(key >> 16) & 0xFFFFu, o[1], P.grid_len));
        f[7] = mz;
        double a[6];
#pragma unroll
        for (int k = 0; k < 6; ++k) {
          float sc = (float)me.s[k];
          if (P.normalize_cov) sc = __fdiv_rn(sc, (float)count);
          f[8 + k] = sc;
          a[k] = (double)sc;
        }
        double w[3], Vv[3][3];
        eig3_sym(a, w, Vv);
        const float e0 = (float)w[0], e1 = (float)w[1], e2 = (float)w[2];
        int k;
        if (e0 < e1) k = (e0 < e2) ? 0 : 2; else k = (e1 < e2) ? 1 : 2;
        float rough = (float)w[k];
        if (rough == 0.f) rough = 0.01f;
        double s0 = w[0], s1 = w[1], s2 = w[2], t;
        if (s0 > s1) { t = s0; s0 = s1; s1 = t; }
        if (s1 > s2) { t = s1; s1 = s2; s2 = t; }
        if (s0 > s1) { t = s0; s0 = s1; s1 = t; }
        f[14] = (float)s0; f[15] = (float)s1; f[16] = (float)s2;
        f[17] = (float)(k == 0 ? Vv[0][0] : (k == 1 ? Vv[0][1] : Vv[0][2]));
        f[18] = (float)(k == 0 ? Vv[1][0] : (k == 1 ? Vv[1][1] : Vv[1][2]));
        f[19] = (float)(k == 0 ? Vv[2][0] : (k == 1 ? Vv[2][1] : Vv[2][2]));
        f[20] = rough;
      }
      u[21] = flags;
#pragma unroll
      for (int i = 0; i < 6; ++i) S.out[tid * 6 + i] = make_float4(f[4 * i], f[4 * i + 1], f[4 * i + 2], f[4 * i + 3]);
      vfirst[v] = first;
    }
    const u32 fitted_cnt = __syncthreads_count(live && fitted);
    if (tid == 0 && fitted_cnt) atomicAdd(&ctl->n_fitted, fitted_cnt);

    if (live) {
      const u32 cols_before = (u32)(S.prefix >> 31) + (exc >> 16);
      const u32 slopes_before = (u32)(S.prefix & 0x7FFFFFFFu) + (exc & 0xFFFFu);
      const u32 col_idx = cols_before + (head ? 1u : 0u) - 1u;
      float4 *rec = S.out + tid * 6;
      float4 last = rec[5];
      last.z = __uint_as_float(col_idx);
      last.w = __uint_as_float(slope ? slopes_before : 0xFFFFFFFFu);
      rec[5] = last;
      if (slope || head) {
        const float4 r0 = rec[0], r1 = rec[1];
        if (slope) {
          const float4 r4 = rec[4];
          float4 *d = reinterpret_cast<float4 *>(slopes + slopes_before);
          d[0] = make_float4(r0.x, r0.y, r0.z, r1.y);
          d[1] = make_float4(r1.z, r1.w, r4.y, r4.z);
          d[2] = make_float4(r4.w, last.x, __uint_as_float(flags), __uint_as_float(v));
          slope_col[slopes_before] = col_idx;
        }
        if (head) {
          float4 *d = reinterpret_cast<float4 *>(columns + col_idx);
          d[0] = make_float4(r0.x, r0.y, r1.x, __uint_as_float(v));
          d[1] = make_float4(0.f, __uint_as_float(slopes_before), 0.f, 0.f);
        }
      }
    }
    tma_store_fence();
    __syncthreads();
    if (tid == 0) {
      tma_store_1d(table + v0, S.out, cnt * (u32)sizeof(gndt_voxel));
      tma_store_wait_read();
    }
  }
}

__global__ void column_finish_kernel(Ctl *ctl, const u32 *vfirst, gndt_column *columns, u32 *row_start, u32 *row_end) {
  pdl_wait();
  pdl_trigger();
  const u32 V = ctl->n_voxels, C = ctl->n_columns, S = ctl->n_slopes;
  const int cx_min = ctl->cx_min, cx_max = ctl->cx_max;
  for (u32 c = blockIdx.x * blockDim.x + threadIdx.x; c < C; c += gridDim.x * blockDim.x) {
    gndt_column col = columns[c];
    const u32 v_end = (c + 1 < C) ? columns[c + 1].voxel_begin : V;
    const u32 s_end = (c + 1 < C) ? columns[c + 1].slope_begin : S;
    u32 first = 0xFFFFFFFFu;
    for (u32 v = col.voxel_begin; v < v_end; ++v) first = min(first, vfirst[v]);
    columns[c].first_index = first;
    columns[c].voxel_count = v_end - col.voxel_begin;
    columns[c].slope_count = s_end - col.slope_begin;
    const int cx = contiguous_index(col.sx);
    if (c == 0 || contiguous_index(columns[c - 1].sx) != cx) {
      row_start[cx - cx_min] = c;
      if (cx == cx_max) ctl->last_row_begin = col.voxel_begin;
    }
    if (c + 1 == C || contiguous_index(columns[c + 1].sx) != cx) {
      row_end[cx - cx_min] = c + 1;
      if (cx == cx_min) ctl->first_row_end = v_end;
    }
  }
}

__device__ __forceinline__ double normal_length(const float a[3]) {
  return sqrt(__dadd_rn(__dadd_rn(__dmul_rn((double)a[0], (double)a[0]), __dmul_rn((double)a[1], (double)a[1])),
                        __dmul_rn((double)a[2], (double)a[2])));
}
__device__ __forceinline__ float count_angle(const float a[3], const float b[3], double l2) {
  float dot = __fmul_rn(a[0], b[0]);
  dot = __fadd_rn(dot, __fmul_rn(a[1], b[1]));
  dot = __fadd_rn(dot, __fmul_rn(a[2], b[2]));
  const double l1 = normal_length(a);
  const float res = (float)((double)dot / __dmul_rn(l1, l2));
  const float deg = __fmul_rn(acosf(res), 180.f);
  float an = (float)((double)deg / 3.14159265358979323846);
  if (an > 90.f) an = __fsub_rn(180.f, an);
  return an;
}

__device__ __forceinline__ bool reachable(const float tn[3], float rough, float tz, u32 flags, const float n[3], double n_len,
                                          float mz, const DevParams &P) {
  return !(flags & GNDT_F_UP) && rough <= P.rough_max && fabsf(__fsub_rn(tz, mz)) <= P.reach_height &&
         count_angle(tn, n, n_len) <= P.angle_max_deg;
}

__device__ __forceinline__ bool cell_reachable(const gndt_column &c, const gndt_slope *slopes, const float n[3],
                                               double n_len, float mz, const DevParams &P) {
  for (u32 s = c.slope_begin; s < c.slope_begin + c.slope_count; ++s) {
    const gndt_slope &t = slopes[s];
    if (reachable(t.normal, t.rough, t.mean[2], t.flags, n, n_len, mz, P)) return true;
  }
  return false;
}

__global__ void __launch_bounds__(256)
edges_kernel(Ctl *ctl, gndt_voxel *table, gndt_slope *slopes, const gndt_column *columns, const u32 *slope_col,
             const u32 *row_start, const u32 *row_end, DevParams P) {
  pdl_wait();
  pdl_trigger();
  const u32 S = ctl->n_slopes, C = ctl->n_columns;
  const int cx_base = ctl->cx_min, cx_max = ctl->cx_max;
  for (u32 i = blockIdx.x * blockDim.x + threadIdx.x; i < S; i += gridDim.x * blockDim.x) {
    gndt_slope me = slopes[i];
    const int cx = contiguous_index(me.sx), cy = contiguous_index(me.sy);
    const u32 ci = slope_col[i];
    const float n[3] = {me.normal[0], me.normal[1], me.normal[2]};
    const double n_len = normal_length(n);
    u32 bits = 0;
    if (ci > 0) {
      const gndt_column c = columns[ci - 1];
      if (contiguous_index(c.sx) == cx && contiguous_index(c.sy) == cy - 1 && cell_reachable(c, slopes, n, n_len, me.mean[2], P))
        bits |= GNDT_F_REACH_L;
    }
    if (ci + 1 < C) {
      const gndt_column c = columns[ci + 1];
      if (contiguous_index(c.sx) == cx && contiguous_index(c.sy) == cy + 1 && cell_reachable(c, slopes, n, n_len, me.mean[2], P))
        bits |= GNDT_F_REACH_R;
    }
#pragma unroll
    for (int dir = 0; dir < 2; ++dir) {
      const int ncx = cx + (dir == 0 ? 1 : -1);
      if (ncx < cx_base || ncx > cx_max) continue;
      const u32 r_lo = row_start[ncx - cx_base], r_hi = row_end[ncx - cx_base];
      u32 lo = r_lo, hi = r_hi;
      if (r_lo < r_hi) {
        const u32 g = r_lo + min(ci - row_start[cx - cx_base], r_hi - r_lo - 1u);
        if (contiguous_index(columns[g].sy) < cy) {
          lo = g + 1;
          for (u32 step = 1;; step <<= 1) {
            const u32 probe = lo + step - 1;
            if (probe >= r_hi) { hi = r_hi; break; }
            if (contiguous_index(columns[probe].sy) >= cy) { hi = probe; break; }
            lo = probe + 1;
          }
        } else {
          hi = g;
          for (u32 step = 1;; step <<= 1) {
            if (hi < r_lo + step) { lo = r_lo; break; }
            const u32 probe = hi - step;
            if (contiguous_index(columns[probe].sy) < cy) { lo = probe + 1; break; }
            hi = probe;
          }
        }
      }
      while (lo < hi) {
        const u32 mid = (lo + hi) >> 1;
        if (contiguous_index(columns[mid].sy) < cy) lo = mid + 1; else hi = mid;
      }
      if (lo < row_end[ncx - cx_base]) {
        const gndt_column c = columns[lo];
        if (contiguous_index(c.sy) == cy && cell_reachable(c, slopes, n, n_len, me.mean[2], P))
          bits |= (dir == 0 ? GNDT_F_REACH_F : GNDT_F_REACH_B);
      }
    }
    if (bits) {
      slopes[i].flags = me.flags | bits;
      table[me.voxel].flags |= bits;
    }
  }
}

}
```

grid_ndt_b200/csrc/gndt_reduce.cuh:

```cuda
#pragma once
#include "gndt_device.cuh"

namespace gndt {

constexpr int kRedThreads = 256;
constexpr int kRedMinBlocks = 5;
constexpr int kRedItems = 8;
constexpr int kRedTile = kRedThreads * kRedItems;
constexpr int kLongRun = 64;
constexpr int kMaxLong = kRedTile / kLongRun;

struct Moments {
  double n;
  double m[3];
  double s[6];
};

struct __align__(16) VoxMoments {
  u64 key;
  u32 count;
  u32 first;
  double m[3];
  double s[6];
  u64 pad;
};

__device__ __forceinline__ double anchor_axis(u32 biased, float o, float len) {
  return __fma_rn((double)((int)biased - kIdxBias) + 0.5, (double)len, (double)o);
}
__device__ __forceinline__ void cell_anchor(u64 key, const float o[3], float grid_len, float z_len, double a[3]) {
  a[0] = anchor_axis((u32)(key >> 32), o[0], grid_len);
  a[1] = anchor_axis((u32)(key >> 16) & 0xFFFFu, o[1], grid_len);
  a[2] = anchor_axis((u32)key & 0xFFFFu, o[2], z_len);
}

constexpr u32 kCarryHasLead = 1u, kCarryLeadContinues = 2u, kCarryHasTail = 4u;
struct TileCarry {
  u32 flags;
  u32 tail_slot;
  u32 pad[2];
  Moments lead;
};

__device__ __forceinline__ void merge_moments(Moments &a, const Moments &b) {
  if (b.n == 0.0) return;
  if (a.n == 0.0) { a = b; return; }
  const double n = a.n + b.n;
  const double d0 = b.m[0] - a.m[0], d1 = b.m[1] - a.m[1], d2 = b.m[2] - a.m[2];
  const double w = a.n * b.n / n, f = b.n / n;
  a.s[0] += b.s[0] + d0 * d0 * w; a.s[1] += b.s[1] + d0 * d1 * w; a.s[2] += b.s[2] + d0 * d2 * w;
  a.s[3] += b.s[3] + d1 * d1 * w; a.s[4] += b.s[4] + d1 * d2 * w; a.s[5] += b.s[5] + d2 * d2 * w;
  a.m[0] += d0 * f; a.m[1] += d1 * f; a.m[2] += d2 * f;
  a.n = n;
}

__device__ __forceinline__ void close_moments(Moments &mo, double n, const float4 &p0, const double anc[3],
                                              const double sd[3], const double sq[6]) {
  const double inv = 1.0 / n;
  const double m0 = sd[0] * inv, m1 = sd[1] * inv, m2 = sd[2] * inv;
  mo.n = n;
  mo.m[0] = ((double)p0.x - anc[0]) + m0; mo.m[1] = ((double)p0.y - anc[1]) + m1; mo.m[2] = ((double)p0.z - anc[2]) + m2;
  mo.s[0] = sq[0] - sd[0] * m0; mo.s[1] = sq[1] - sd[0] * m1; mo.s[2] = sq[2] - sd[0] * m2;
  mo.s[3] = sq[3] - sd[1] * m1; mo.s[4] = sq[4] - sd[1] * m2; mo.s[5] = sq[5] - sd[2] * m2;
}

__device__ __forceinline__ void sym2(double &app, double &aqq, double apq, double &c, double &s) {
  const double theta = (aqq - app) / (2.0 * apq);
  const double t = (theta >= 0 ? 1.0 : -1.0) / (fabs(theta) + sqrt(theta * theta + 1.0));
  c = 1.0 / sqrt(t * t + 1.0);
  s = t * c;
  app -= t * apq;
  aqq += t * apq;
}

__device__ void eig3_sym(const double a[6], double w[3], double V[3][3]) {
  const double a00 = a[0], a01 = a[1], a02 = a[2], a11 = a[3], a12 = a[4], a22 = a[5];
#pragma unroll
  for (int i = 0; i < 3; ++i)
#pragma unroll
    for (int j = 0; j < 3; ++j) V[i][j] = (i == j) ? 1.0 : 0.0;
  w[0] = a00; w[1] = a11; w[2] = a22;
  const int nz = (a01 != 0.0) + (a02 != 0.0) + (a12 != 0.0);
  if (nz == 0) return;
  if (nz == 1) {
    double c, s;
    if (a01 != 0.0) {
      sym2(w[0], w[1], a01, c, s);
      V[0][0] = c; V[1][0] = -s; V[0][1] = s; V[1][1] = c;
    } else if (a02 != 0.0) {
      sym2(w[0], w[2], a02, c, s);
      V[0][0] = c; V[2][0] = -s; V[0][2] = s; V[2][2] = c;
    } else {
      sym2(w[1], w[2], a12, c, s);
      V[1][1] = c; V[2][1] = -s; V[1][2] = s; V[2][2] = c;
    }
    return;
  }
  double sc = fmax(fmax(fabs(a00), fabs(a11)), fabs(a22));
  sc = fmax(sc, fmax(fmax(fabs(a01), fabs(a02)), fabs(a12)));
  const double inv = 1.0 / sc;
  const double b00 = a00 * inv, b01 = a01 * inv, b02 = a02 * inv, b11 = a11 * inv, b12 = a12 * inv, b22 = a22 * inv;
  const double q = (b00 + b11 + b22) / 3.0;
  const double c00 = b00 - q, c11 = b11 - q, c22 = b22 - q;
  const double p2 = c00 * c00 + c11 * c11 + c22 * c22 + 2.0 * (b01 * b01 + b02 * b02 + b12 * b12);
  const double p = sqrt(p2 / 6.0);
  const double ip = 1.0 / p;
  const double d00 = c00 * ip, d11 = c11 * ip, d22 = c22 * ip, d01 = b01 * ip, d02 = b02 * ip, d12 = b12 * ip;
  double r = 0.5 * (d00 * (d11 * d22 - d12 * d12) - d01 * (d01 * d22 - d12 * d02) + d02 * (d01 * d12 - d11 * d02));
  r = fmin(1.0, fmax(-1.0, r));
  const double phi = acos(r) / 3.0;
  const double e_max = q + 2.0 * p * cos(phi);
  const double e_min = q + 2.0 * p * cos(phi + 2.0943951023931954923);
  const double e_mid = 3.0 * q - e_max - e_min;
  const double ev[3] = {e_min, e_mid, e_max};
#pragma unroll
  for (int k = 0; k < 3; ++k) {
    const double l = ev[k];
    const double r0[3] = {b00 - l, b01, b02}, r1[3] = {b01, b11 - l, b12}, r2[3] = {b02, b12, b22 - l};
    double x0[3] = {r0[1] * r1[2] - r0[2] * r1[1], r0[2] * r1[0] - r0[0] * r1[2], r0[0] * r1[1] - r0[1] * r1[0]};
    double x1[3] = {r0[1] * r2[2] - r0[2] * r2[1], r0[2] * r2[0] - r0[0] * r2[2], r0[0] * r2[1] - r0[1] * r2[0]};
    double x2[3] = {r1[1] * r2[2] - r1[2] * r2[1], r1[2] * r2[0] - r1[0] * r2[2], r1[0] * r2[1] - r1[1] * r2[0]};
    const double n0 = x0[0] * x0[0] + x0[1] * x0[1] + x0[2] * x0[2];
    const double n1 = x1[0] * x1[0] + x1[1] * x1[1] + x1[2] * x1[2];
    const double n2 = x2[0] * x2[0] + x2[1] * x2[1] + x2[2] * x2[2];
    double bx = x0[0], by = x0[1], bz = x0[2], bn = n0;
    if (n1 > bn) { bx = x1[0]; by = x1[1]; bz = x1[2]; bn = n1; }
    if (n2 > bn) { bx = x2[0]; by = x2[1]; bz = x2[2]; bn = n2; }
    if (bn > 0.0) {
      const double in = rsqrt(bn);
      V[0][k] = bx * in; V[1][k] = by * in; V[2][k] = bz * in;
    } else {
      V[0][k] = (k == 0); V[1][k] = (k == 1); V[2][k] = (k == 2);
    }
    w[k] = l * sc;
  }
}

struct __align__(128) RedSmem {
  float4 pts_raw[kRedTile + 2];
  unsigned long long mbar;
  unsigned short run_start[kRedTile + 2];
  unsigned short long_list[kMaxLong];
  u64 row_last_key[kRedItems][8];
  u32 seg_cnt[kRedItems][8];
  double red[8][9];
  u64 prev_key, next_key, first_key, last_key;
  u32 n_long, tile_id, n_runs, vox_base;
};

template <bool FAST>
__device__ __forceinline__ u64 point_key(const float4 &p, const float o[3], const DevParams &P) {
  int cx, cy, cz;
  point_indices_masked_t<FAST>(p.x, p.y, p.z, o, P, 7, cx, cy, cz);
  return voxel_key(cx, cy, cz);
}

__device__ __forceinline__ void store_moments(VoxMoments *dst, u64 key, u32 first, const Moments &mo) {
  VoxMoments v;
  v.key = key; v.count = (u32)mo.n; v.first = first;
#pragma unroll
  for (int k = 0; k < 3; ++k) v.m[k] = mo.m[k];
#pragma unroll
  for (int k = 0; k < 6; ++k) v.s[k] = mo.s[k];
  v.pad = 0;
  const double2 *q = reinterpret_cast<const double2 *>(&v);
  double2 *d = reinterpret_cast<double2 *>(dst);
#pragma unroll
  for (int i = 0; i < 6; ++i) d[i] = q[i];
}

template <bool FAST>
__global__ void __launch_bounds__(kRedThreads, kRedMinBlocks)
reduce_kernel(Ctl *ctl, const float4 *buf_a, const float4 *buf_b, VoxMoments *mom, TileCarry *carry,
              u64 *tile_state, GroupState *tile_groups, DevParams P) {
  pdl_wait();
  pdl_trigger();
  extern __shared__ __align__(16) unsigned char smem_raw[];
  RedSmem &S = *reinterpret_cast<RedSmem *>(smem_raw);
  const int tid = threadIdx.x, lane = tid & 31, warp = tid >> 5;
  if (tid == 0) { S.tile_id = atomicAdd(&ctl->ticket[6], 1u); S.n_long = 0; mbar_init(&S.mbar, 1); }
  __syncthreads();
  const int tile = (int)S.tile_id;
  const size_t M = (size_t)ctl->n_valid;
  const size_t base = (size_t)tile * kRedTile;
  if (base >= M) return;
  const int cnt = (int)min((size_t)kRedTile, M - base);
  const float4 *src = ((ctl->n_passes - 1) & 1) ? buf_b : buf_a;
  const float o[3] = {ctl->origin[0], ctl->origin[1], ctl->origin[2]};
  float4 *pts = S.pts_raw + 1;

  const bool has_prev = base > 0, has_next = base + cnt < M;
  if (tid == 0)
    tma_load_1d(S.pts_raw + (has_prev ? 0 : 1), src + base - (has_prev ? 1 : 0),
                (u32)(cnt + (has_prev ? 1 : 0) + (has_next ? 1 : 0)) * 16u, &S.mbar);
  if (!mbar_wait(&S.mbar, 0)) atomicOr(&ctl->err, kErrWatchdog);
  u64 key[kRedItems];
#pragma unroll
  for (int k = 0; k < kRedItems; ++k) {
    const int i = k * kRedThreads + tid;
    key[k] = ~0ull;
    if (i < cnt) key[k] = point_key<FAST>(pts[i], o, P);
    if (lane == 31) S.row_last_key[k][warp] = key[k];
    if (i == 0) S.first_key = key[k];
    if (i == cnt - 1) S.last_key = key[k];
  }
  if (tid == 0) S.prev_key = has_prev ? point_key<FAST>(S.pts_raw[0], o, P) : ~0ull;
  if (tid == 32) S.next_key = has_next ? point_key<FAST>(pts[cnt], o, P) : ~0ull;
  __syncthreads();

  u32 ball[kRedItems];
#pragma unroll
  for (int k = 0; k < kRedItems; ++k) {
    const int i = k * kRedThreads + tid;
    u64 before = __shfl_up_sync(0xffffffffu, key[k], 1);
    if (lane == 0) before = (warp > 0) ? S.row_last_key[k][warp - 1] : (k > 0 ? S.row_last_key[k - 1][7] : ~key[k]);
    const bool head = (i < cnt) && (i == 0 || key[k] != before);
    ball[k] = __ballot_sync(0xffffffffu, head);
    if (lane == 0) S.seg_cnt[k][warp] = __popc(ball[k]);
  }
  __syncthreads();
  if (warp == 0) {
    u32 c0 = (&S.seg_cnt[0][0])[2 * lane], c1 = (&S.seg_cnt[0][0])[2 * lane + 1];
    u32 inc = c0 + c1;
#pragma unroll
    for (int o2 = 1; o2 < 32; o2 <<= 1) {
      u32 t = __shfl_up_sync(0xffffffffu, inc, o2);
      if (lane >= o2) inc += t;
    }
    const u32 exc = inc - (c0 + c1);
    (&S.seg_cnt[0][0])[2 * lane] = exc;
    (&S.seg_cnt[0][0])[2 * lane + 1] = exc + c0;
    if (lane == 31) S.n_runs = inc;
  }
  __syncthreads();
#pragma unroll
  for (int k = 0; k < kRedItems; ++k) {
    const int i = k * kRedThreads + tid;
    if (ball[k] & (1u << lane)) S.run_start[S.seg_cnt[k][warp] + __popc(ball[k] & ((1u << lane) - 1u))] = (unsigned short)i;
  }
  const int n_runs = (int)S.n_runs;
  const bool first_is_head = S.prev_key != S.first_key;
  const bool last_complete = S.next_key != S.last_key;
  const u32 heads = (u32)n_runs - (first_is_head ? 0u : 1u);
  if (tid == 0) S.run_start[n_runs] = (unsigned short)cnt;
  __syncthreads();

  auto run_moments = [&](int j, Moments &mo, u64 &key) -> bool {
    const int s = S.run_start[j], e = S.run_start[j + 1];
    if (e - s > kLongRun) {
      S.long_list[atomicAdd(&S.n_long, 1u)] = (unsigned short)j;
      return false;
    }
    const float4 p0 = pts[s];
    key = point_key<FAST>(p0, o, P);
    double anc[3];
    cell_anchor(key, o, P.grid_len, P.z_len, anc);
    double sd[3] = {0, 0, 0}, sq[6] = {0, 0, 0, 0, 0, 0};
    for (int i = s + 1; i < e; ++i) {
      const float4 p = pts[i];
      const double dx = (double)p.x - (double)p0.x, dy = (double)p.y - (double)p0.y, dz = (double)p.z - (double)p0.z;
      sd[0] += dx; sd[1] += dy; sd[2] += dz;
      sq[0] += dx * dx; sq[1] += dx * dy; sq[2] += dx * dz; sq[3] += dy * dy; sq[4] += dy * dz; sq[5] += dz * dz;
    }
    close_moments(mo, (double)(e - s), p0, anc, sd, sq);
    return true;
  };
  Moments mo0;
  u64 key0;
  const bool have0 = (tid < n_runs) && run_moments(tid, mo0, key0);

  if (warp == kRedThreads / 32 - 1) {
    const u64 vb = warp_lookback_grouped(tile_state, tile_groups, tile, 0u, heads, &ctl->err);
    if (lane == 0) S.vox_base = (u32)vb;
  }
  __syncthreads();
  const u32 vox_base = S.vox_base;
  if (tid == 0 && base + cnt == M) ctl->n_voxels = vox_base + heads;
  TileCarry *my_carry = carry + tile;

  auto emit = [&](int j, const Moments &mo, u64 key) {
    const int s = S.run_start[j];
    const bool cont = (j == 0) && !first_is_head;
    const bool open_end = (j == n_runs - 1) && !last_complete;
    const u32 slot = vox_base + (u32)j - (first_is_head ? 0u : 1u);
    if (cont) {
      my_carry->lead = mo;
      atomicOr(&my_carry->flags, kCarryHasLead | (open_end ? kCarryLeadContinues : 0u));
      return;
    }
    if (slot >= P.max_voxels) { atomicOr(&ctl->err, kErrCapacity); return; }
    store_moments(mom + slot, key, __float_as_uint(pts[s].w), mo);
    if (open_end) {
      my_carry->tail_slot = slot;
      atomicOr(&my_carry->flags, kCarryHasTail);
    }
  };
  if (have0) emit(tid, mo0, key0);
  for (int j = tid + kRedThreads; j < n_runs; j += kRedThreads) {
    Moments mo;
    u64 key;
    if (run_moments(j, mo, key)) emit(j, mo, key);
  }
  __syncthreads();

  const int n_long = (int)S.n_long;
  for (int l = warp; l < n_long; l += kRedThreads / 32) {
    const int j = S.long_list[l];
    const int s = S.run_start[j], e = S.run_start[j + 1];
    const float4 p0 = pts[s];
    double acc[9] = {0, 0, 0, 0, 0, 0, 0, 0, 0};
    for (int i = s + lane; i < e; i += 32) {
      const float4 p = pts[i];
      const double dx = (double)p.x - (double)p0.x, dy = (double)p.y - (double)p0.y, dz = (double)p.z - (double)p0.z;
      acc[0] += dx; acc[1] += dy; acc[2] += dz;
      acc[3] += dx * dx; acc[4] += dx * dy; acc[5] += dx * dz; acc[6] += dy * dy; acc[7] += dy * dz; acc[8] += dz * dz;
    }
#pragma unroll
    for (int k = 0; k < 9; ++k) acc[k] = warp_sum(acc[k]);
    if (lane == 0) {
      const u64 key = point_key<FAST>(p0, o, P);
      double anc[3];
      cell_anchor(key, o, P.grid_len, P.z_len, anc);
      Moments mo;
      close_moments(mo, (double)(e - s), p0, anc, acc, acc + 3);
      emit(j, mo, key);
    }
  }
}

__global__ void __launch_bounds__(128) fixup_kernel(Ctl *ctl, VoxMoments *mom, const TileCarry *carry) {
  pdl_wait();
  pdl_trigger();
  const size_t M = (size_t)ctl->n_valid;
  const int n_tiles = (int)((M + kRedTile - 1) / kRedTile);
  const int lane = threadIdx.x & 31;
  const int warps_total = (gridDim.x * blockDim.x) >> 5;
  for (int t = (blockIdx.x * blockDim.x + threadIdx.x) >> 5; t < n_tiles; t += warps_total) {
    if (!(carry[t].flags & kCarryHasTail)) continue;
    Moments acc;
    acc.n = 0.0;
#pragma unroll
    for (int k = 0; k < 3; ++k) acc.m[k] = 0.0;
#pragma unroll
    for (int k = 0; k < 6; ++k) acc.s[k] = 0.0;
    for (int u0 = t + 1; u0 < n_tiles; u0 += 32) {
      const int u = u0 + lane;
      const u32 fl = (u < n_tiles) ? carry[u].flags : 0u;
      const u32 has_lead = __ballot_sync(0xffffffffu, (fl & kCarryHasLead) != 0);
      const u32 ends_here = __ballot_sync(0xffffffffu, (fl & kCarryHasLead) && !(fl & kCarryLeadContinues));
      const int stop_excl = (~has_lead) ? __ffs(~has_lead) - 1 : 32;
      const int stop_incl = ends_here ? __ffs(ends_here) : 33;
      const int n_inc = min(stop_excl, stop_incl);
      Moments mine;
      mine.n = 0.0;
#pragma unroll
      for (int k = 0; k < 3; ++k) mine.m[k] = 0.0;
#pragma unroll
      for (int k = 0; k < 6; ++k) mine.s[k] = 0.0;
      if (lane < n_inc) mine = carry[u].lead;
#pragma unroll
      for (int o = 1; o < 32; o <<= 1) {
        Moments other;
        other.n = __shfl_down_sync(0xffffffffu, mine.n, o);
#pragma unroll
        for (int k = 0; k < 3; ++k) other.m[k] = __shfl_down_sync(0xffffffffu, mine.m[k], o);
#pragma unroll
        for (int k = 0; k < 6; ++k) other.s[k] = __shfl_down_sync(0xffffffffu, mine.s[k], o);
        if (lane + o < 32) merge_moments(mine, other);
      }
      if (lane == 0) merge_moments(acc, mine);
      if (n_inc < 32 || ends_here) break;
    }
    if (lane == 0) {
      VoxMoments *v = mom + carry[t].tail_slot;
      Moments mo;
      mo.n = (double)v->count;
#pragma unroll
      for (int k = 0; k < 3; ++k) mo.m[k] = v->m[k];
#pragma unroll
      for (int k = 0; k < 6; ++k) mo.s[k] = v->s[k];
      merge_moments(mo, acc);
      v->count = (u32)mo.n;
#pragma unroll
      for (int k = 0; k < 3; ++k) v->m[k] = mo.m[k];
#pragma unroll
      for (int k = 0; k < 6; ++k) v->s[k] = mo.s[k];
    }
  }
}

}
```

Before: 15.69 billion.

## Fuse cross-tile moment fixup into reduce kernel via decoupled lookback carries

For the build path, the reduce kernel now publishes each tile's boundary lead and tail moments before the lookback. The tile that closes a voxel spanning several tiles merges the chain itself and writes the final moments, so the separate fixup kernel launch is dropped. The update path keeps the old reduce-plus-fixup flow. Shared moment helpers move into a new header and the short/long run loops become functions. This removes one kernel launch and a global pass over the carries, at the cost of extra fences and serialized boundary work in the last warp before the lookback.

```diff
diff --git a/grid_ndt_b200/_lib.py b/grid_ndt_b200/_lib.py
--- a/grid_ndt_b200/_lib.py
+++ b/grid_ndt_b200/_lib.py
@@ -9,7 +9,7 @@
 REPO = os.path.dirname(HERE)
 LIB_PATH = os.environ.get("GNDT_LIB") or os.path.join(HERE, "libgndt.so")
 SOURCES = [os.path.join(HERE, "csrc", f) for f in (
-    "gndt_api.cu", "gndt_device.cuh", "gndt_sort.cuh", "gndt_reduce.cuh", "gndt_label.cuh", "gndt_update.cuh",
+    "gndt_api.cu", "gndt_device.cuh", "gndt_sort.cuh", "gndt_moments.cuh", "gndt_reduce.cuh", "gndt_label.cuh", "gndt_update.cuh",
     "gndt_exchange.cuh", "gndt_graph.cuh", "gndt_scan.cuh", "gndt_ndt.cuh")]
 HEADER = os.path.join(REPO, "include", "gndt.h")
 LOOKUP_HEADER = os.path.join(REPO, "include", "gndt_lookup.h")
diff --git a/grid_ndt_b200/csrc/gndt_api.cu b/grid_ndt_b200/csrc/gndt_api.cu
--- a/grid_ndt_b200/csrc/gndt_api.cu
+++ b/grid_ndt_b200/csrc/gndt_api.cu
@@ -81,6 +81,7 @@
   TileCarry *carry = nullptr;
   u64 *blk_state = nullptr;
   GroupState *blk_groups = nullptr;
+  VoxMoments *tails = nullptr;
   size_t zero_bytes_used = 0;
   size_t sort_tiles = 0, sort_groups = 0, red_tiles = 0, label_blocks = 0;
   Buffer f_zero;
@@ -341,11 +342,13 @@
   Layout B;
   const size_t lb_bytes = h->sort_tiles * kMaxBins * sizeof(u32) + 256, glb_bytes = h->sort_groups * kMaxBins * sizeof(u64) + 256;
   const size_t o_lb[2] = {B.take(lb_bytes), B.take(lb_bytes)}, o_glb[2] = {B.take(glb_bytes), B.take(glb_bytes)};
+  const size_t o_tt = B.take(h->red_tiles * sizeof(VoxMoments));
   if ((rc = ensure(h, h->lookback, B.bytes)) != GNDT_OK) return rc;
   for (int k = 0; k < 2; ++k) {
     h->lb[k] = at<u32>(h->lookback, o_lb[k]);
     h->glb[k] = at<u64>(h->lookback, o_glb[k]);
   }
+  h->tails = at<VoxMoments>(h->lookback, o_tt);
   return GNDT_OK;
 }
 
@@ -394,7 +397,7 @@
 }
 
 int front_end(gndt_handle *h, cudaStream_t st, const float *d_in, size_t n, size_t stride_f, size_t start,
-              const DevParams &dp, VoxMoments *out) {
+              const DevParams &dp, VoxMoments *out, bool merge) {
   GNDT_CUDA(h, cudaMemsetAsync(h->zero.p, 0, h->zero_bytes_used, st));
   const size_t tiles = (n + kSortTile - 1) / kSortTile, groups = (tiles + kSortGroup - 1) / kSortGroup;
   auto *bounds = dp.fast_div ? bounds_kernel<true> : bounds_kernel<false>;
@@ -417,10 +420,16 @@
   }
   if (h->stage_timing) GNDT_CUDA(h, cudaEventRecord(h->ev[EV_SORT], st));
   const int rtiles = (int)((n + kRedTile - 1) / kRedTile);
-  auto *reduce = dp.fast_div ? reduce_kernel<true> : reduce_kernel<false>;
-  launch(h, true, reduce, rtiles, kRedThreads, sizeof(RedSmem), st, h->ctl, (const float4 *)A, (const float4 *)B, out, h->carry,
-         h->tile_state, h->tile_groups, dp);
-  launch(h, true, fixup_kernel, grid_for(h, (size_t)rtiles * 32, 128, 16), 128, 0, st, h->ctl, out, (const TileCarry *)h->carry);
+  if (merge) {
+    auto *reduce = dp.fast_div ? reduce_kernel<true, true> : reduce_kernel<false, true>;
+    launch(h, true, reduce, rtiles, kRedThreads, sizeof(RedSmem), st, h->ctl, (const float4 *)A, (const float4 *)B, out, h->carry,
+           h->tile_state, h->tile_groups, h->tails, dp);
+  } else {
+    auto *reduce = dp.fast_div ? reduce_kernel<true, false> : reduce_kernel<false, false>;
+    launch(h, true, reduce, rtiles, kRedThreads, sizeof(RedSmem), st, h->ctl, (const float4 *)A, (const float4 *)B, out, h->carry,
+           h->tile_state, h->tile_groups, (VoxMoments *)nullptr, dp);
+    launch(h, true, fixup_kernel, grid_for(h, (size_t)rtiles * 32, 128, 16), 128, 0, st, h->ctl, out, (const TileCarry *)h->carry);
+  }
   if (h->stage_timing) GNDT_CUDA(h, cudaEventRecord(h->ev[EV_REDUCE], st));
   return GNDT_OK;
 }
@@ -498,8 +507,10 @@
   if (e == cudaSuccess) e = cudaFuncSetAttribute(sort_pass_kernel<true, false>, cudaFuncAttributeMaxDynamicSharedMemorySize, (int)sizeof(SortSmem));
   if (e == cudaSuccess) e = cudaFuncSetAttribute(sort_pass_kernel<false, true>, cudaFuncAttributeMaxDynamicSharedMemorySize, (int)sizeof(SortSmem));
   if (e == cudaSuccess) e = cudaFuncSetAttribute(sort_pass_kernel<false, false>, cudaFuncAttributeMaxDynamicSharedMemorySize, (int)sizeof(SortSmem));
-  if (e == cudaSuccess) e = cudaFuncSetAttribute(reduce_kernel<true>, cudaFuncAttributeMaxDynamicSharedMemorySize, (int)sizeof(RedSmem));
-  if (e == cudaSuccess) e = cudaFuncSetAttribute(reduce_kernel<false>, cudaFuncAttributeMaxDynamicSharedMemorySize, (int)sizeof(RedSmem));
+  if (e == cudaSuccess) e = cudaFuncSetAttribute(reduce_kernel<true, false>, cudaFuncAttributeMaxDynamicSharedMemorySize, (int)sizeof(RedSmem));
+  if (e == cudaSuccess) e = cudaFuncSetAttribute(reduce_kernel<false, false>, cudaFuncAttributeMaxDynamicSharedMemorySize, (int)sizeof(RedSmem));
+  if (e == cudaSuccess) e = cudaFuncSetAttribute(reduce_kernel<true, true>, cudaFuncAttributeMaxDynamicSharedMemorySize, (int)sizeof(RedSmem));
+  if (e == cudaSuccess) e = cudaFuncSetAttribute(reduce_kernel<false, true>, cudaFuncAttributeMaxDynamicSharedMemorySize, (int)sizeof(RedSmem));
   if (e == cudaSuccess) e = cudaFuncSetAttribute(finalize_label_kernel, cudaFuncAttributeMaxDynamicSharedMemorySize, (int)sizeof(FinSmem));
   if (e != cudaSuccess) { g_create_error = std::string("kernel image for sm_100a not loadable on this device: ") + cudaGetErrorString(e); delete h; return GNDT_ERR_CUDA; }
   for (int k = 0; k < 2; ++k) {
@@ -551,7 +562,7 @@
   const DevParams dp = make_dev(h, h->params, h->cap_voxels);
   h->ndt_ready = false;
   GNDT_CUDA(h, cudaEventRecord(h->ev[EV_START], st));
-  int rc = front_end(h, st, d_in, n, stride_bytes / 4, start, dp, (VoxMoments *)h->mom.p);
+  int rc = front_end(h, st, d_in, n, stride_bytes / 4, start, dp, (VoxMoments *)h->mom.p, true);
   if (rc != GNDT_OK) return rc;
   launch(h, true, totals_kernel, 1, 32, 0, st, &static_cast<SmallWords *>(h->small.p)->tot, (const Ctl *)h->ctl, (u64)n, 1, 1);
   rc = back_end(h, st, dp, (const VoxMoments *)h->mom.p, false);
@@ -715,7 +726,7 @@
 
   GNDT_CUDA(h, cudaEventRecord(h->ev[EV_START], st));
   VoxMoments *res = (VoxMoments *)h->mom.p, *scan = (VoxMoments *)h->mom_scan.p, *merged = (VoxMoments *)h->mom_alt.p;
-  rc = front_end(h, st, d_in, n, stride_bytes / 4, 0, dp, scan);
+  rc = front_end(h, st, d_in, n, stride_bytes / 4, 0, dp, scan, false);
   if (rc != GNDT_OK) return rc;
   SmallWords *small = static_cast<SmallWords *>(h->small.p);
   launch(h, false, totals_kernel, 1, 32, 0, st, &small->tot, h->ctl, (u64)n, 0, sign);
diff --git a/grid_ndt_b200/csrc/gndt_label.cuh b/grid_ndt_b200/csrc/gndt_label.cuh
--- a/grid_ndt_b200/csrc/gndt_label.cuh
+++ b/grid_ndt_b200/csrc/gndt_label.cuh
@@ -1,6 +1,6 @@
 #pragma once
 #include "gndt_device.cuh"
-#include "gndt_reduce.cuh"
+#include "gndt_moments.cuh"
 
 namespace gndt {
 
diff --git a/grid_ndt_b200/csrc/gndt_moments.cuh b/grid_ndt_b200/csrc/gndt_moments.cuh
--- /dev/null
+++ b/grid_ndt_b200/csrc/gndt_moments.cuh
@@ -0,0 +1,124 @@
+#pragma once
+#include "gndt_device.cuh"
+
+namespace gndt {
+
+struct Moments {
+  double n;
+  double m[3];
+  double s[6];
+};
+
+struct __align__(16) VoxMoments {
+  u64 key;
+  u32 count;
+  u32 first;
+  double m[3];
+  double s[6];
+  u64 pad;
+};
+
+__device__ __forceinline__ double anchor_axis(u32 biased, float o, float len) {
+  return __fma_rn((double)((int)biased - kIdxBias) + 0.5, (double)len, (double)o);
+}
+__device__ __forceinline__ void cell_anchor(u64 key, const float o[3], float grid_len, float z_len, double a[3]) {
+  a[0] = anchor_axis((u32)(key >> 32), o[0], grid_len);
+  a[1] = anchor_axis((u32)(key >> 16) & 0xFFFFu, o[1], grid_len);
+  a[2] = anchor_axis((u32)key & 0xFFFFu, o[2], z_len);
+}
+
+__device__ __forceinline__ void merge_moments(Moments &a, const Moments &b) {
+  if (b.n == 0.0) return;
+  if (a.n == 0.0) { a = b; return; }
+  const double n = a.n + b.n;
+  const double d0 = b.m[0] - a.m[0], d1 = b.m[1] - a.m[1], d2 = b.m[2] - a.m[2];
+  const double w = a.n * b.n / n, f = b.n / n;
+  a.s[0] += b.s[0] + d0 * d0 * w; a.s[1] += b.s[1] + d0 * d1 * w; a.s[2] += b.s[2] + d0 * d2 * w;
+  a.s[3] += b.s[3] + d1 * d1 * w; a.s[4] += b.s[4] + d1 * d2 * w; a.s[5] += b.s[5] + d2 * d2 * w;
+  a.m[0] += d0 * f; a.m[1] += d1 * f; a.m[2] += d2 * f;
+  a.n = n;
+}
+
+__device__ __forceinline__ void close_moments(Moments &mo, double n, const float4 &p0, const double anc[3],
+                                              const double sd[3], const double sq[6]) {
+  const double inv = 1.0 / n;
+  const double m0 = sd[0] * inv, m1 = sd[1] * inv, m2 = sd[2] * inv;
+  mo.n = n;
+  mo.m[0] = ((double)p0.x - anc[0]) + m0; mo.m[1] = ((double)p0.y - anc[1]) + m1; mo.m[2] = ((double)p0.z - anc[2]) + m2;
+  mo.s[0] = sq[0] - sd[0] * m0; mo.s[1] = sq[1] - sd[0] * m1; mo.s[2] = sq[2] - sd[0] * m2;
+  mo.s[3] = sq[3] - sd[1] * m1; mo.s[4] = sq[4] - sd[1] * m2; mo.s[5] = sq[5] - sd[2] * m2;
+}
+
+__device__ __forceinline__ void sym2(double &app, double &aqq, double apq, double &c, double &s) {
+  const double theta = (aqq - app) / (2.0 * apq);
+  const double t = (theta >= 0 ? 1.0 : -1.0) / (fabs(theta) + sqrt(theta * theta + 1.0));
+  c = 1.0 / sqrt(t * t + 1.0);
+  s = t * c;
+  app -= t * apq;
+  aqq += t * apq;
+}
+
+__device__ void eig3_sym(const double a[6], double w[3], double V[3][3]) {
+  const double a00 = a[0], a01 = a[1], a02 = a[2], a11 = a[3], a12 = a[4], a22 = a[5];
+#pragma unroll
+  for (int i = 0; i < 3; ++i)
+#pragma unroll
+    for (int j = 0; j < 3; ++j) V[i][j] = (i == j) ? 1.0 : 0.0;
+  w[0] = a00; w[1] = a11; w[2] = a22;
+  const int nz = (a01 != 0.0) + (a02 != 0.0) + (a12 != 0.0);
+  if (nz == 0) return;
+  if (nz == 1) {
+    double c, s;
+    if (a01 != 0.0) {
+      sym2(w[0], w[1], a01, c, s);
+      V[0][0] = c; V[1][0] = -s; V[0][1] = s; V[1][1] = c;
+    } else if (a02 != 0.0) {
+      sym2(w[0], w[2], a02, c, s);
+      V[0][0] = c; V[2][0] = -s; V[0][2] = s; V[2][2] = c;
+    } else {
+      sym2(w[1], w[2], a12, c, s);
+      V[1][1] = c; V[2][1] = -s; V[1][2] = s; V[2][2] = c;
+    }
+    return;
+  }
+  double sc = fmax(fmax(fabs(a00), fabs(a11)), fabs(a22));
+  sc = fmax(sc, fmax(fmax(fabs(a01), fabs(a02)), fabs(a12)));
+  const double inv = 1.0 / sc;
+  const double b00 = a00 * inv, b01 = a01 * inv, b02 = a02 * inv, b11 = a11 * inv, b12 = a12 * inv, b22 = a22 * inv;
+  const double q = (b00 + b11 + b22) / 3.0;
+  const double c00 = b00 - q, c11 = b11 - q, c22 = b22 - q;
+  const double p2 = c00 * c00 + c11 * c11 + c22 * c22 + 2.0 * (b01 * b01 + b02 * b02 + b12 * b12);
+  const double p = sqrt(p2 / 6.0);
+  const double ip = 1.0 / p;
+  const double d00 = c00 * ip, d11 = c11 * ip, d22 = c22 * ip, d01 = b01 * ip, d02 = b02 * ip, d12 = b12 * ip;
+  double r = 0.5 * (d00 * (d11 * d22 - d12 * d12) - d01 * (d01 * d22 - d12 * d02) + d02 * (d01 * d12 - d11 * d02));
+  r = fmin(1.0, fmax(-1.0, r));
+  const double phi = acos(r) / 3.0;
+  const double e_max = q + 2.0 * p * cos(phi);
+  const double e_min = q + 2.0 * p * cos(phi + 2.0943951023931954923);
+  const double e_mid = 3.0 * q - e_max - e_min;
+  const double ev[3] = {e_min, e_mid, e_max};
+#pragma unroll
+  for (int k = 0; k < 3; ++k) {
+    const double l = ev[k];
+    const double r0[3] = {b00 - l, b01, b02}, r1[3] = {b01, b11 - l, b12}, r2[3] = {b02, b12, b22 - l};
+    double x0[3] = {r0[1] * r1[2] - r0[2] * r1[1], r0[2] * r1[0] - r0[0] * r1[2], r0[0] * r1[1] - r0[1] * r1[0]};
+    double x1[3] = {r0[1] * r2[2] - r0[2] * r2[1], r0[2] * r2[0] - r0[0] * r2[2], r0[0] * r2[1] - r0[1] * r2[0]};
+    double x2[3] = {r1[1] * r2[2] - r1[2] * r2[1], r1[2] * r2[0] - r1[0] * r2[2], r1[0] * r2[1] - r1[1] * r2[0]};
+    const double n0 = x0[0] * x0[0] + x0[1] * x0[1] + x0[2] * x0[2];
+    const double n1 = x1[0] * x1[0] + x1[1] * x1[1] + x1[2] * x1[2];
+    const double n2 = x2[0] * x2[0] + x2[1] * x2[1] + x2[2] * x2[2];
+    double bx = x0[0], by = x0[1], bz = x0[2], bn = n0;
+    if (n1 > bn) { bx = x1[0]; by = x1[1]; bz = x1[2]; bn = n1; }
+    if (n2 > bn) { bx = x2[0]; by = x2[1]; bz = x2[2]; bn = n2; }
+    if (bn > 0.0) {
+      const double in = rsqrt(bn);
+      V[0][k] = bx * in; V[1][k] = by * in; V[2][k] = bz * in;
+    } else {
+      V[0][k] = (k == 0); V[1][k] = (k == 1); V[2][k] = (k == 2);
+    }
+    w[k] = l * sc;
+  }
+}
+
+}
diff --git a/grid_ndt_b200/csrc/gndt_reduce.cuh b/grid_ndt_b200/csrc/gndt_reduce.cuh
--- a/grid_ndt_b200/csrc/gndt_reduce.cuh
+++ b/grid_ndt_b200/csrc/gndt_reduce.cuh
@@ -1,5 +1,6 @@
 #pragma once
 #include "gndt_device.cuh"
+#include "gndt_moments.cuh"
 
 namespace gndt {
 
@@ -9,30 +10,6 @@
 constexpr int kRedTile = kRedThreads * kRedItems;
 constexpr int kLongRun = 64;
 constexpr int kMaxLong = kRedTile / kLongRun;
-
-struct Moments {
-  double n;
-  double m[3];
-  double s[6];
-};
-
-struct __align__(16) VoxMoments {
-  u64 key;
-  u32 count;
-  u32 first;
-  double m[3];
-  double s[6];
-  u64 pad;
-};
-
-__device__ __forceinline__ double anchor_axis(u32 biased, float o, float len) {
-  return __fma_rn((double)((int)biased - kIdxBias) + 0.5, (double)len, (double)o);
-}
-__device__ __forceinline__ void cell_anchor(u64 key, const float o[3], float grid_len, float z_len, double a[3]) {
-  a[0] = anchor_axis((u32)(key >> 32), o[0], grid_len);
-  a[1] = anchor_axis((u32)(key >> 16) & 0xFFFFu, o[1], grid_len);
-  a[2] = anchor_axis((u32)key & 0xFFFFu, o[2], z_len);
-}
 
 constexpr u32 kCarryHasLead = 1u, kCarryLeadContinues = 2u, kCarryHasTail = 4u;
 struct TileCarry {
@@ -41,101 +18,6 @@
   u32 pad[2];
   Moments lead;
 };
-
-__device__ __forceinline__ void merge_moments(Moments &a, const Moments &b) {
-  if (b.n == 0.0) return;
-  if (a.n == 0.0) { a = b; return; }
-  const double n = a.n + b.n;
-  const double d0 = b.m[0] - a.m[0], d1 = b.m[1] - a.m[1], d2 = b.m[2] - a.m[2];
-  const double w = a.n * b.n / n, f = b.n / n;
-  a.s[0] += b.s[0] + d0 * d0 * w; a.s[1] += b.s[1] + d0 * d1 * w; a.s[2] += b.s[2] + d0 * d2 * w;
-  a.s[3] += b.s[3] + d1 * d1 * w; a.s[4] += b.s[4] + d1 * d2 * w; a.s[5] += b.s[5] + d2 * d2 * w;
-  a.m[0] += d0 * f; a.m[1] += d1 * f; a.m[2] += d2 * f;
-  a.n = n;
-}
-
-__device__ __forceinline__ void close_moments(Moments &mo, double n, const float4 &p0, const double anc[3],
-                                              const double sd[3], const double sq[6]) {
-  const double inv = 1.0 / n;
-  const double m0 = sd[0] * inv, m1 = sd[1] * inv, m2 = sd[2] * inv;
-  mo.n = n;
-  mo.m[0] = ((double)p0.x - anc[0]) + m0; mo.m[1] = ((double)p0.y - anc[1]) + m1; mo.m[2] = ((double)p0.z - anc[2]) + m2;
-  mo.s[0] = sq[0] - sd[0] * m0; mo.s[1] = sq[1] - sd[0] * m1; mo.s[2] = sq[2] - sd[0] * m2;
-  mo.s[3] = sq[3] - sd[1] * m1; mo.s[4] = sq[4] - sd[1] * m2; mo.s[5] = sq[5] - sd[2] * m2;
-}
-
-__device__ __forceinline__ void sym2(double &app, double &aqq, double apq, double &c, double &s) {
-  const double theta = (aqq - app) / (2.0 * apq);
-  const double t = (theta >= 0 ? 1.0 : -1.0) / (fabs(theta) + sqrt(theta * theta + 1.0));
-  c = 1.0 / sqrt(t * t + 1.0);
-  s = t * c;
-  app -= t * apq;
-  aqq += t * apq;
-}
-
-__device__ void eig3_sym(const double a[6], double w[3], double V[3][3]) {
-  const double a00 = a[0], a01 = a[1], a02 = a[2], a11 = a[3], a12 = a[4], a22 = a[5];
-#pragma unroll
-  for (int i = 0; i < 3; ++i)
-#pragma unroll
-    for (int j = 0; j < 3; ++j) V[i][j] = (i == j) ? 1.0 : 0.0;
-  w[0] = a00; w[1] = a11; w[2] = a22;
-  const int nz = (a01 != 0.0) + (a02 != 0.0) + (a12 != 0.0);
-  if (nz == 0) return;
-  if (nz == 1) {
-    double c, s;
-    if (a01 != 0.0) {
-      sym2(w[0], w[1], a01, c, s);
-      V[0][0] = c; V[1][0] = -s; V[0][1] = s; V[1][1] = c;
-    } else if (a02 != 0.0) {
-      sym2(w[0], w[2], a02, c, s);
-      V[0][0] = c; V[2][0] = -s; V[0][2] = s; V[2][2] = c;
-    } else {
-      sym2(w[1], w[2], a12, c, s);
-      V[1][1] = c; V[2][1] = -s; V[1][2] = s; V[2][2] = c;
-    }
-    return;
-  }
-  double sc = fmax(fmax(fabs(a00), fabs(a11)), fabs(a22));
-  sc = fmax(sc, fmax(fmax(fabs(a01), fabs(a02)), fabs(a12)));
-  const double inv = 1.0 / sc;
-  const double b00 = a00 * inv, b01 = a01 * inv, b02 = a02 * inv, b11 = a11 * inv, b12 = a12 * inv, b22 = a22 * inv;
-  const double q = (b00 + b11 + b22) / 3.0;
-  const double c00 = b00 - q, c11 = b11 - q, c22 = b22 - q;
-  const double p2 = c00 * c00 + c11 * c11 + c22 * c22 + 2.0 * (b01 * b01 + b02 * b02 + b12 * b12);
-  const double p = sqrt(p2 / 6.0);
-  const double ip = 1.0 / p;
-  const double d00 = c00 * ip, d11 = c11 * ip, d22 = c22 * ip, d01 = b01 * ip, d02 = b02 * ip, d12 = b12 * ip;
-  double r = 0.5 * (d00 * (d11 * d22 - d12 * d12) - d01 * (d01 * d22 - d12 * d02) + d02 * (d01 * d12 - d11 * d02));
-  r = fmin(1.0, fmax(-1.0, r));
-  const double phi = acos(r) / 3.0;
-  const double e_max = q + 2.0 * p * cos(phi);
-  const double e_min = q + 2.0 * p * cos(phi + 2.0943951023931954923);
-  const double e_mid = 3.0 * q - e_max - e_min;
-  const double ev[3] = {e_min, e_mid, e_max};
-#pragma unroll
-  for (int k = 0; k < 3; ++k) {
-    const double l = ev[k];
-    const double r0[3] = {b00 - l, b01, b02}, r1[3] = {b01, b11 - l, b12}, r2[3] = {b02, b12, b22 - l};
-    double x0[3] = {r0[1] * r1[2] - r0[2] * r1[1], r0[2] * r1[0] - r0[0] * r1[2], r0[0] * r1[1] - r0[1] * r1[0]};
-    double x1[3] = {r0[1] * r2[2] - r0[2] * r2[1], r0[2] * r2[0] - r0[0] * r2[2], r0[0] * r2[1] - r0[1] * r2[0]};
-    double x2[3] = {r1[1] * r2[2] - r1[2] * r2[1], r1[2] * r2[0] - r1[0] * r2[2], r1[0] * r2[1] - r1[1] * r2[0]};
-    const double n0 = x0[0] * x0[0] + x0[1] * x0[1] + x0[2] * x0[2];
-    const double n1 = x1[0] * x1[0] + x1[1] * x1[1] + x1[2] * x1[2];
-    const double n2 = x2[0] * x2[0] + x2[1] * x2[1] + x2[2] * x2[2];
-    double bx = x0[0], by = x0[1], bz = x0[2], bn = n0;
-    if (n1 > bn) { bx = x1[0]; by = x1[1]; bz = x1[2]; bn = n1; }
-    if (n2 > bn) { bx = x2[0]; by = x2[1]; bz = x2[2]; bn = n2; }
-    if (bn > 0.0) {
-      const double in = rsqrt(bn);
-      V[0][k] = bx * in; V[1][k] = by * in; V[2][k] = bz * in;
-    } else {
-      V[0][k] = (k == 0); V[1][k] = (k == 1); V[2][k] = (k == 2);
-    }
-    w[k] = l * sc;
-  }
-}
-
 struct __align__(128) RedSmem {
   float4 pts_raw[kRedTile + 2];
   unsigned long long mbar;
@@ -155,7 +37,7 @@
   return voxel_key(cx, cy, cz);
 }
 
-__device__ __forceinline__ void store_moments(VoxMoments *dst, u64 key, u32 first, const Moments &mo) {
+__device__ __forceinline__ VoxMoments vox_record(u64 key, u32 first, const Moments &mo) {
   VoxMoments v;
   v.key = key; v.count = (u32)mo.n; v.first = first;
 #pragma unroll
@@ -163,16 +45,133 @@
 #pragma unroll
   for (int k = 0; k < 6; ++k) v.s[k] = mo.s[k];
   v.pad = 0;
+  return v;
+}
+__device__ __forceinline__ void store_vox(VoxMoments *dst, const VoxMoments &v) {
   const double2 *q = reinterpret_cast<const double2 *>(&v);
   double2 *d = reinterpret_cast<double2 *>(dst);
 #pragma unroll
   for (int i = 0; i < 6; ++i) d[i] = q[i];
 }
+__device__ __forceinline__ void store_moments(VoxMoments *dst, u64 key, u32 first, const Moments &mo) {
+  store_vox(dst, vox_record(key, first, mo));
+}
+__device__ __forceinline__ VoxMoments load_vox_cg(const VoxMoments *p) {
+  VoxMoments v;
+  double2 *q = reinterpret_cast<double2 *>(&v);
+#pragma unroll
+  for (int i = 0; i < 6; ++i) q[i] = __ldcg(reinterpret_cast<const double2 *>(p) + i);
+  return v;
+}
+__device__ __forceinline__ Moments load_moments_cg(const Moments *p) {
+  Moments m;
+  m.n = __ldcg(&p->n);
+#pragma unroll
+  for (int k = 0; k < 3; ++k) m.m[k] = __ldcg(&p->m[k]);
+#pragma unroll
+  for (int k = 0; k < 6; ++k) m.s[k] = __ldcg(&p->s[k]);
+  return m;
+}
 
 template <bool FAST>
+__device__ __forceinline__ void short_run(const float4 *pts, int s, int e, const float o[3], const DevParams &P, Moments &mo, u64 &key) {
+  const float4 p0 = pts[s];
+  key = point_key<FAST>(p0, o, P);
+  double anc[3];
+  cell_anchor(key, o, P.grid_len, P.z_len, anc);
+  double sd[3] = {0, 0, 0}, sq[6] = {0, 0, 0, 0, 0, 0};
+  for (int i = s + 1; i < e; ++i) {
+    const float4 p = pts[i];
+    const double dx = (double)p.x - (double)p0.x, dy = (double)p.y - (double)p0.y, dz = (double)p.z - (double)p0.z;
+    sd[0] += dx; sd[1] += dy; sd[2] += dz;
+    sq[0] += dx * dx; sq[1] += dx * dy; sq[2] += dx * dz; sq[3] += dy * dy; sq[4] += dy * dz; sq[5] += dz * dz;
+  }
+  close_moments(mo, (double)(e - s), p0, anc, sd, sq);
+}
+template <bool FAST>
+__device__ __forceinline__ void long_run(const float4 *pts, int s, int e, const float o[3], const DevParams &P, Moments &mo, u64 &key) {
+  const int lane = threadIdx.x & 31;
+  const float4 p0 = pts[s];
+  double acc[9] = {0, 0, 0, 0, 0, 0, 0, 0, 0};
+  for (int i = s + lane; i < e; i += 32) {
+    const float4 p = pts[i];
+    const double dx = (double)p.x - (double)p0.x, dy = (double)p.y - (double)p0.y, dz = (double)p.z - (double)p0.z;
+    acc[0] += dx; acc[1] += dy; acc[2] += dz;
+    acc[3] += dx * dx; acc[4] += dx * dy; acc[5] += dx * dz; acc[6] += dy * dy; acc[7] += dy * dz; acc[8] += dz * dz;
+  }
+#pragma unroll
+  for (int k = 0; k < 9; ++k) acc[k] = warp_sum(acc[k]);
+  key = point_key<FAST>(p0, o, P);
+  double anc[3];
+  cell_anchor(key, o, P.grid_len, P.z_len, anc);
+  close_moments(mo, (double)(e - s), p0, anc, acc, acc + 3);
+}
+
+__device__ __forceinline__ Moments merge_leads(const TileCarry *carry, int t, int last) {
+  const int lane = threadIdx.x & 31;
+  Moments acc;
+  acc.n = 0.0;
+#pragma unroll
+  for (int k = 0; k < 3; ++k) acc.m[k] = 0.0;
+#pragma unroll
+  for (int k = 0; k < 6; ++k) acc.s[k] = 0.0;
+  for (int u0 = t + 1; u0 <= last; u0 += 32) {
+    const int u = u0 + lane;
+    const u32 fl = (u <= last) ? __ldcg(&carry[u].flags) : 0u;
+    const u32 has_lead = __ballot_sync(0xffffffffu, (fl & kCarryHasLead) != 0);
+    const u32 ends_here = __ballot_sync(0xffffffffu, (fl & kCarryHasLead) && !(fl & kCarryLeadContinues));
+    const int stop_excl = (~has_lead) ? __ffs(~has_lead) - 1 : 32;
+    const int stop_incl = ends_here ? __ffs(ends_here) : 33;
+    const int n_inc = min(stop_excl, stop_incl);
+    Moments mine;
+    mine.n = 0.0;
+#pragma unroll
+    for (int k = 0; k < 3; ++k) mine.m[k] = 0.0;
+#pragma unroll
+    for (int k = 0; k < 6; ++k) mine.s[k] = 0.0;
+    if (lane < n_inc) mine = load_moments_cg(&carry[u].lead);
+#pragma unroll
+    for (int o = 1; o < 32; o <<= 1) {
+      Moments other;
+      other.n = __shfl_down_sync(0xffffffffu, mine.n, o);
+#pragma unroll
+      for (int k = 0; k < 3; ++k) other.m[k] = __shfl_down_sync(0xffffffffu, mine.m[k], o);
+#pragma unroll
+      for (int k = 0; k < 6; ++k) other.s[k] = __shfl_down_sync(0xffffffffu, mine.s[k], o);
+      if (lane + o < 32) merge_moments(mine, other);
+    }
+    if (lane == 0) merge_moments(acc, mine);
+    if (n_inc < 32 || ends_here) break;
+  }
+  return acc;
+}
+
+__device__ __forceinline__ int chain_head(const TileCarry *carry, int e) {
+  const int lane = threadIdx.x & 31;
+  for (int hi = e - 1;; hi -= 32) {
+    const int u = hi - lane;
+    const u32 fl = (u >= 0) ? __ldcg(&carry[u].flags) : 0u;
+    const u32 stop = __ballot_sync(0xffffffffu, !((fl & kCarryHasLead) && (fl & kCarryLeadContinues)));
+    if (stop) return hi - (__ffs(stop) - 1);
+  }
+}
+__device__ __forceinline__ VoxMoments chain_voxel(const TileCarry *carry, const VoxMoments *tails, int t, int e) {
+  const Moments acc = merge_leads(carry, t, e);
+  const VoxMoments tv = load_vox_cg(tails + t);
+  Moments mo;
+  mo.n = (double)tv.count;
+#pragma unroll
+  for (int k = 0; k < 3; ++k) mo.m[k] = tv.m[k];
+#pragma unroll
+  for (int k = 0; k < 6; ++k) mo.s[k] = tv.s[k];
+  merge_moments(mo, acc);
+  return vox_record(tv.key, tv.first, mo);
+}
+
+template <bool FAST, bool MERGE>
 __global__ void __launch_bounds__(kRedThreads, kRedMinBlocks)
 reduce_kernel(Ctl *ctl, const float4 *buf_a, const float4 *buf_b, VoxMoments *mom, TileCarry *carry,
-              u64 *tile_state, GroupState *tile_groups, DevParams P) {
+              u64 *tile_state, GroupState *tile_groups, VoxMoments *tails, DevParams P) {
   pdl_wait();
   pdl_trigger();
   extern __shared__ __align__(16) unsigned char smem_raw[];
@@ -185,11 +184,12 @@
   const size_t base = (size_t)tile * kRedTile;
   if (base >= M) return;
   const int cnt = (int)min((size_t)kRedTile, M - base);
+  const bool is_last = base + cnt == M;
   const float4 *src = ((ctl->n_passes - 1) & 1) ? buf_b : buf_a;
   const float o[3] = {ctl->origin[0], ctl->origin[1], ctl->origin[2]};
   float4 *pts = S.pts_raw + 1;
 
-  const bool has_prev = base > 0, has_next = base + cnt < M;
+  const bool has_prev = base > 0, has_next = !is_last;
   if (tid == 0)
     tma_load_1d(S.pts_raw + (has_prev ? 0 : 1), src + base - (has_prev ? 1 : 0),
                 (u32)(cnt + (has_prev ? 1 : 0) + (has_next ? 1 : 0)) * 16u, &S.mbar);
@@ -251,18 +251,7 @@
       S.long_list[atomicAdd(&S.n_long, 1u)] = (unsigned short)j;
       return false;
     }
-    const float4 p0 = pts[s];
-    key = point_key<FAST>(p0, o, P);
-    double anc[3];
-    cell_anchor(key, o, P.grid_len, P.z_len, anc);
-    double sd[3] = {0, 0, 0}, sq[6] = {0, 0, 0, 0, 0, 0};
-    for (int i = s + 1; i < e; ++i) {
-      const float4 p = pts[i];
-      const double dx = (double)p.x - (double)p0.x, dy = (double)p.y - (double)p0.y, dz = (double)p.z - (double)p0.z;
-      sd[0] += dx; sd[1] += dy; sd[2] += dz;
-      sq[0] += dx * dx; sq[1] += dx * dy; sq[2] += dx * dz; sq[3] += dy * dy; sq[4] += dy * dz; sq[5] += dz * dz;
-    }
-    close_moments(mo, (double)(e - s), p0, anc, sd, sq);
+    short_run<FAST>(pts, s, e, o, P, mo, key);
     return true;
   };
   Moments mo0;
@@ -270,12 +259,42 @@
   const bool have0 = (tid < n_runs) && run_moments(tid, mo0, key0);
 
   if (warp == kRedThreads / 32 - 1) {
+    if constexpr (MERGE) {
+      const bool has_lead = !first_is_head, has_tail = !last_complete && (n_runs > 1 || first_is_head);
+      int j = -1;
+      if (lane == 0 && has_lead) j = 0;
+      if (lane == 1 && has_tail) j = n_runs - 1;
+      Moments mo;
+      u64 k = 0;
+      if (j >= 0 && S.run_start[j + 1] - S.run_start[j] <= kLongRun) short_run<FAST>(pts, S.run_start[j], S.run_start[j + 1], o, P, mo, k);
+#pragma unroll 1
+      for (int c = 0; c < 2; ++c) {
+        const int jc = __shfl_sync(0xffffffffu, j, c);
+        if (jc >= 0 && S.run_start[jc + 1] - S.run_start[jc] > kLongRun) {
+          Moments ml;
+          u64 kl;
+          long_run<FAST>(pts, S.run_start[jc], S.run_start[jc + 1], o, P, ml, kl);
+          if (lane == c) { mo = ml; k = kl; }
+        }
+      }
+      if (lane == 0 && j >= 0) carry[tile].lead = mo;
+      if (lane == 1 && j >= 0) store_vox(tails + tile, vox_record(k, __float_as_uint(pts[S.run_start[j]].w), mo));
+      if (lane == 0) {
+        carry[tile].flags = (has_lead ? kCarryHasLead | (n_runs == 1 && !last_complete ? kCarryLeadContinues : 0u) : 0u) |
+                            (has_tail ? kCarryHasTail : 0u);
+      }
+      __threadfence();
+      __syncwarp();
+    }
     const u64 vb = warp_lookback_grouped(tile_state, tile_groups, tile, 0u, heads, &ctl->err);
     if (lane == 0) S.vox_base = (u32)vb;
+    if constexpr (MERGE) {
+      __threadfence();
+    }
   }
   __syncthreads();
   const u32 vox_base = S.vox_base;
-  if (tid == 0 && base + cnt == M) ctl->n_voxels = vox_base + heads;
+  if (tid == 0 && is_last) ctl->n_voxels = vox_base + heads;
   TileCarry *my_carry = carry + tile;
 
   auto emit = [&](int j, const Moments &mo, u64 key) {
@@ -284,15 +303,22 @@
     const bool open_end = (j == n_runs - 1) && !last_complete;
     const u32 slot = vox_base + (u32)j - (first_is_head ? 0u : 1u);
     if (cont) {
-      my_carry->lead = mo;
-      atomicOr(&my_carry->flags, kCarryHasLead | (open_end ? kCarryLeadContinues : 0u));
+      if constexpr (!MERGE) {
+        my_carry->lead = mo;
+        atomicOr(&my_carry->flags, kCarryHasLead | (open_end ? kCarryLeadContinues : 0u));
+      }
       return;
     }
     if (slot >= P.max_voxels) { atomicOr(&ctl->err, kErrCapacity); return; }
-    store_moments(mom + slot, key, __float_as_uint(pts[s].w), mo);
-    if (open_end) {
-      my_carry->tail_slot = slot;
-      atomicOr(&my_carry->flags, kCarryHasTail);
+    if constexpr (MERGE) {
+      if (open_end) return;
+      store_moments(mom + slot, key, __float_as_uint(pts[s].w), mo);
+    } else {
+      store_moments(mom + slot, key, __float_as_uint(pts[s].w), mo);
+      if (open_end) {
+        my_carry->tail_slot = slot;
+        atomicOr(&my_carry->flags, kCarryHasTail);
+      }
     }
   };
   if (have0) emit(tid, mo0, key0);
@@ -303,28 +329,19 @@
   }
   __syncthreads();
 
+  if constexpr (MERGE) {
+    if (warp == kRedThreads / 32 - 1 && !first_is_head && (n_runs > 1 || last_complete)) {
+      const VoxMoments v = chain_voxel(carry, tails, chain_head(carry, tile), tile);
+      if (lane == 0 && vox_base - 1 < P.max_voxels) store_vox(mom + (vox_base - 1), v);
+    }
+  }
   const int n_long = (int)S.n_long;
   for (int l = warp; l < n_long; l += kRedThreads / 32) {
     const int j = S.long_list[l];
-    const int s = S.run_start[j], e = S.run_start[j + 1];
-    const float4 p0 = pts[s];
-    double acc[9] = {0, 0, 0, 0, 0, 0, 0, 0, 0};
-    for (int i = s + lane; i < e; i += 32) {
-      const float4 p = pts[i];
-      const double dx = (double)p.x - (double)p0.x, dy = (double)p.y - (double)p0.y, dz = (double)p.z - (double)p0.z;
-      acc[0] += dx; acc[1] += dy; acc[2] += dz;
-      acc[3] += dx * dx; acc[4] += dx * dy; acc[5] += dx * dz; acc[6] += dy * dy; acc[7] += dy * dz; acc[8] += dz * dz;
-    }
-#pragma unroll
-    for (int k = 0; k < 9; ++k) acc[k] = warp_sum(acc[k]);
-    if (lane == 0) {
-      const u64 key = point_key<FAST>(p0, o, P);
-      double anc[3];
-      cell_anchor(key, o, P.grid_len, P.z_len, anc);
-      Moments mo;
-      close_moments(mo, (double)(e - s), p0, anc, acc, acc + 3);
-      emit(j, mo, key);
-    }
+    Moments mo;
+    u64 key;
+    long_run<FAST>(pts, S.run_start[j], S.run_start[j + 1], o, P, mo, key);
+    if (lane == 0) emit(j, mo, key);
   }
 }
 
@@ -337,40 +354,7 @@
   const int warps_total = (gridDim.x * blockDim.x) >> 5;
   for (int t = (blockIdx.x * blockDim.x + threadIdx.x) >> 5; t < n_tiles; t += warps_total) {
     if (!(carry[t].flags & kCarryHasTail)) continue;
-    Moments acc;
-    acc.n = 0.0;
-#pragma unroll
-    for (int k = 0; k < 3; ++k) acc.m[k] = 0.0;
-#pragma unroll
-    for (int k = 0; k < 6; ++k) acc.s[k] = 0.0;
-    for (int u0 = t + 1; u0 < n_tiles; u0 += 32) {
-      const int u = u0 + lane;
-      const u32 fl = (u < n_tiles) ? carry[u].flags : 0u;
-      const u32 has_lead = __ballot_sync(0xffffffffu, (fl & kCarryHasLead) != 0);
-      const u32 ends_here = __ballot_sync(0xffffffffu, (fl & kCarryHasLead) && !(fl & kCarryLeadContinues));
-      const int stop_excl = (~has_lead) ? __ffs(~has_lead) - 1 : 32;
-      const int stop_incl = ends_here ? __ffs(ends_here) : 33;
-      const int n_inc = min(stop_excl, stop_incl);
-      Moments mine;
-      mine.n = 0.0;
-#pragma unroll
-      for (int k = 0; k < 3; ++k) mine.m[k] = 0.0;
-#pragma unroll
-      for (int k = 0; k < 6; ++k) mine.s[k] = 0.0;
-      if (lane < n_inc) mine = carry[u].lead;
-#pragma unroll
-      for (int o = 1; o < 32; o <<= 1) {
-        Moments other;
-        other.n = __shfl_down_sync(0xffffffffu, mine.n, o);
-#pragma unroll
-        for (int k = 0; k < 3; ++k) other.m[k] = __shfl_down_sync(0xffffffffu, mine.m[k], o);
-#pragma unroll
-        for (int k = 0; k < 6; ++k) other.s[k] = __shfl_down_sync(0xffffffffu, mine.s[k], o);
-        if (lane + o < 32) merge_moments(mine, other);
-      }
-      if (lane == 0) merge_moments(acc, mine);
-      if (n_inc < 32 || ends_here) break;
-    }
+    const Moments acc = merge_leads(carry, t, n_tiles - 1);
     if (lane == 0) {
       VoxMoments *v = mom + carry[t].tail_slot;
       Moments mo;
```

New measurement: 14.65 billion (median of 6 runs). -6.6%, worse.
